# pedroegsilva/gofindthem

Hardware: AMD Instinct MI355X
Metric: ProcessText throughput: documents/s (and input GB/s), 10000-term dictionary + 1000 expressions, 1000000 docs of ~4 KB sharded over 1 GPU(s) (higher is better)
Workload: dtype u8; 1 GPU; BASELINE.json configs[2]: 10000 terms + 1000 AND/OR/NOT expressions, 1000000 docs x ~4 KB on this GPU (SURVEY.md 8(d) generator), case-insensitive finder, inputs resident in HBM; alphabet=lower, keywords=10000, docs_total=1000000, docs_per_gpu=1000000, text_bytes_per_gpu=4100690990, parallelism=docs sharded x1, cu_margin=0

## Files before the change

### gofindthem_amd/csrc/gft_api.cpp

```cpp
#include "../../include/gft.h"

#include <hip/hip_runtime.h>

#include <algorithm>
#include <chrono>
#include <cstdio>
#include <cstring>
#include <map>
#include <memory>
#include <mutex>
#include <string>
#include <thread>
#include <unordered_set>
#include <vector>

#include <cstdlib>

#include "ac_tables.hpp"
#include "copy_pool.hpp"
#include "gft_guard.hpp"
#include "gft_kernels.hpp"
#include "host_solve.hpp"
#include "scan2_tables.hpp"
#include "scan3_tables.hpp"

using namespace gft;

namespace {

struct DevBuf {
    void* p = nullptr;
    size_t cap = 0;
    hipError_t ensure(size_t bytes) {
        if (bytes <= cap) return hipSuccess;
        if (p) { hipError_t e = hipFree(p); p = nullptr; cap = 0; if (e != hipSuccess) return e; }
        size_t want = bytes + bytes / 8 + 256;
        hipError_t e = hipMalloc(&p, want);
        if (e == hipSuccess) cap = want;
        return e;
    }
    void release() { if (p) (void)hipFree(p); p = nullptr; cap = 0; }
    template <class T> T* as() const { return reinterpret_cast<T*>(p); }
};

struct ProfCat {
    std::vector<std::pair<hipEvent_t, hipEvent_t>> ev;
};

}

#ifndef GFT_EXTRA_KERNELS
namespace gft {
bool scan2_plan(uint32_t, uint32_t, uint32_t, uint32_t, size_t, uint32_t*, uint32_t*) { return false; }
hipError_t launch_scan2(const Scan2Params&, uint32_t, unsigned, hipStream_t) { return hipErrorNotSupported; }
bool scan4_plan(uint32_t, uint32_t, uint32_t, uint32_t, size_t, bool, uint32_t*, uint32_t*) { return false; }
hipError_t launch_scan4(const Scan2Params&, uint32_t, unsigned, hipStream_t) { return hipErrorNotSupported; }
}
static constexpr bool kExtraKernels = false;
#else
static constexpr bool kExtraKernels = true;
#endif

struct gft_engine {
    int device = 0;
    hipStream_t stream = nullptr;
    void* pin[2] = {nullptr, nullptr};
    uint64_t* pin_rb = nullptr;
    hipEvent_t pin_ev[2] = {nullptr, nullptr};
    std::unique_ptr<gft::CopyPool> copy_pool;
    bool own_stream = false;
    unsigned n_cus = 256;
    unsigned n_cus_hw = 256, cu_margin = 0;
    size_t lds_max = 65536;
    mutable std::string err;

    AcTables tab;
    bool built = false;
    uint32_t build_flags = 0;
    uint32_t n_lds_states = 0;
    DevBuf d_byte_class, d_delta, d_out_term, d_out_link, d_term_len;
    Scan2Tables s2;
    bool use_scan2 = false;
    DevBuf d_s2_filter, d_s2_slots, d_s2_more, d_s2_cls, d_s2_cls_fold, d_s2_term_blob, d_s2_term_off, d_dbg;
    Scan3Tables s3;
    bool use_scan3 = false;
    DevBuf d_s3_filter, d_s3_short3, d_s3_srec, d_s3_short3_big, d_s3_srec_big, d_s3_bloom, d_s3_slots, d_s3_more, d_s3_cls,
        d_s3_cls_fold, d_s3_term_blob, d_s3_term_off;
    uint32_t scan3_waves = 0, scan3_cand_cap = 0;
    DevBuf d_ctl;
    DevBuf d_s2_short3, d_s2_shorts_packed, d_s2_short3_big, d_s2_fpt;
    uint32_t scan2_short3_bytes = 0;
    uint32_t scan2_k2_waves = 0, scan2_cand_cap = 0;
    bool use_scan4 = false;
    uint32_t scan4_waves = 0, scan4_fifo[2] = {0, 0};
    double scan4_density = 0.06;
    bool use_scan5 = false;
    Scan5Plan s5plan{0, 0, 0, 0};
    Scan5Tables s5;
    DevBuf d_s5_grp, d_s5_grp_fold, d_s5_filter, d_s5_bloom;
    std::vector<uint32_t> s5_bloom;
    uint32_t s5_bloom_lg = 0;
    uint32_t opt_scan5_bloom_kb = 32;
    uint32_t s5_term_bits = 0, s5_pos_bias = 0;
    bool s5_short_groups = false;
    uint32_t opt_scan5_large = 1;
    uint32_t opt_scan5_fifo = 0;
    uint32_t opt_scan5_groups = 0;
    uint64_t scan_valid_docs = ~0ull;
    uint32_t scan2_unit_max = kScan2UnitMax;
    bool deferred = false;
    uint64_t deferred_unit_cap = 0, deferred_pool_cap = 0;
    uint32_t last_nonascii_bits = 0;
    bool last_nonascii = false;
    uint64_t last_text_lo = 0, last_text_hi = 0;
    uint32_t opt_scan_dbg = 0;
    uint32_t opt_scan_prio = 1;
    uint32_t opt_scan_ordered = 0;
    uint32_t opt_scan4_round = 0;
    uint32_t opt_scan4_chunk = 0;
    uint32_t opt_solve_dbg = 0;
    int opt_solve_group = -1;
    mutable std::recursive_mutex mu;
    std::vector<gft_engine*> peers;
    std::vector<uint64_t> shard_cut;
    bool in_multi = false;
    std::vector<void*> comms;
    bool rccl_self = false;
    void* rccl_lib = nullptr;

    bool have_programs = false;
    uint32_t n_exprs = 0, n_extra = 0;
    std::vector<uint32_t> h_prog;
    std::vector<uint64_t> h_prog_off;
    std::vector<ProgramTraits> traits;
    std::vector<uint32_t> host_only;
    std::vector<uint32_t> inord_exprs;
    std::vector<uint8_t> inord_slot;
    uint64_t last_n_units = 0, last_total = 0;
    bool csr_valid = false;
    DevBuf d_patch;
    DevBuf d_prog, d_prog_off;
    DevBuf d_fprog, d_fprog_off, d_groups;
    DevBuf d_wide_slot, d_wide_theta;
    DevBuf d_solve_dbg;
    int single_streak = 0;
    uint64_t last_static_slabs = 0;
    bool deferred_single = false;
    uint32_t ctl_epoch = 1, deferred_epoch = 0;
    uint64_t deferred_n_docs = 0;
    struct Pending {
        bool done = false;
        int rc = 0;
        const uint8_t* d_text = nullptr; const uint64_t* d_doc_off = nullptr; uint64_t n_docs = 0; uint32_t flags = 0;
        uint32_t* d_bitmap = nullptr;
        bool single = false; uint32_t epoch = 0; uint64_t n_docs_cap = 0, unit_cap = 0, pool_cap = 0, static_slabs = 0;
        uint64_t* rb = nullptr; hipEvent_t ev = nullptr;
        bool nonascii = false; uint32_t nonascii_bits = 0; uint64_t text_lo = 0, text_hi = 0;
    };
    Pending pend[2];
    unsigned pend_head = 0, pend_count = 0;
    DevBuf d_order, d_blk_class, d_wave_blk;
    uint32_t last_solve_group_docs = 64;
    DevBuf d_fprog_t, d_fblk_off;
    uint32_t fprog_words = 0;
    uint32_t n_inord_groups = 0;
    uint32_t wide_pairs = 0;
    uint32_t n_wide = 0;
    DevBuf d_wide_list;
    uint32_t n_rare_words = 0;
    DevBuf d_pscratch;

    DevBuf d_unit_cnt, d_unit_base, d_units, d_partial, d_pool_term, d_pool_pos, d_unit_start,
        d_unit_count, d_unit_out, d_term, d_pos, d_match_off;
    uint64_t pool_cap = 0;
    DevBuf d_text, d_doc_off, d_bitmap, d_xoff, d_xslot, d_xpos;
    DevBuf d_uq_first, d_uq_cnt, d_uq_off, d_uq_term;
    DevBuf d_rn_cnt, d_rn_base, d_rn_starts, d_rn_prefix;
    std::vector<uint64_t> h_match_off;
    std::vector<uint32_t> h_term, h_pos;

    int profiling = 0;
    std::vector<hipEvent_t> prof_pool;
    std::map<std::string, ProfCat> prof;
};

namespace {

void refresh_options(gft_engine* e) {
    auto num = [](const char* name, long dflt) { const char* v = getenv(name); return v ? atol(v) : dflt; };
    e->opt_scan_dbg = (uint32_t)num("GFT_SCAN_DEBUG", 0);
    e->opt_scan_prio = num("GFT_SCAN_PRIO", 1) ? 1u : 0u;
    e->opt_scan_ordered = getenv("GFT_SCAN_ORDERED") ? 1u : 0u;
    e->opt_scan4_chunk = (uint32_t)num("GFT_SCAN4_CHUNK", 0);
    e->opt_scan4_round = (uint32_t)num("GFT_SCAN4_ROUND", 0);
    e->opt_scan5_groups = (uint32_t)num("GFT_SCAN5_GROUPS", 0);
    e->opt_scan5_large = num("GFT_SCAN5_LARGE", 1) ? 1u : 0u;
    e->opt_scan5_bloom_kb = (uint32_t)std::min<long>(std::max<long>(num("GFT_SCAN5_BLOOM_KB", 32), 0), 64);
    e->opt_scan5_fifo = (uint32_t)std::min<long>(std::max<long>(num("GFT_SCAN5_FIFO", 0), 0), 4096) & ~63u;
    e->opt_solve_dbg = (uint32_t)num("GFT_SOLVE_DEBUG", 0);
    e->opt_solve_group = (int)num("GFT_SOLVE_GROUP_DOCS", -1);
}
#define GFT_LOCK(e) std::lock_guard<std::recursive_mutex> _gft_lock((e)->mu)

int fail(const gft_engine* e, int code, const std::string& msg) {
    e->err = msg;
    return code;
}
int fail_hip(const gft_engine* e, hipError_t h, const char* what) {
    e->err = std::string(what) + ": " + hipGetErrorString(h);
    return GFT_E_HIP;
}

#define HIP_TRY(expr, what)                                   \
    do {                                                      \
        hipError_t _h = (expr);                               \
        if (_h != hipSuccess) return fail_hip(e, _h, what);   \
    } while (0)

struct DeviceGuard {
    int prev = -1;
    bool ok = true;
    explicit DeviceGuard(int dev) {
        if (hipGetDevice(&prev) != hipSuccess) prev = -1;
        if (prev != dev) ok = hipSetDevice(dev) == hipSuccess;
    }
    ~DeviceGuard() { if (prev >= 0) (void)hipSetDevice(prev); }
};

struct SyncOnExit {
    gft_engine* e;
    explicit SyncOnExit(gft_engine* e_) : e(e_) {}
    ~SyncOnExit() { if (e->device >= 0 && e->stream) (void)hipStreamSynchronize(e->stream); }
};

struct ProfScope {
    gft_engine* e;
    hipEvent_t a = nullptr, b = nullptr;
    ProfScope(gft_engine* e_, const char* cat) : e(e_) {
        if (!e->profiling || (e->profiling == 2 && std::strcmp(cat, "scan") != 0)) return;
        auto get = [&](hipEvent_t* ev) {
            if (!e->prof_pool.empty()) { *ev = e->prof_pool.back(); e->prof_pool.pop_back(); return true; }
            return hipEventCreate(ev) == hipSuccess;
        };
        if (!get(&a) || !get(&b)) { a = b = nullptr; return; }
        (void)hipEventRecord(a, e->stream);
        e->prof[cat].ev.emplace_back(a, b);
    }
    ~ProfScope() { if (b) (void)hipEventRecord(b, e->stream); }
};

template <class T>
int upload(gft_engine* e, DevBuf& buf, const std::vector<T>& v, const char* what) {
    HIP_TRY(buf.ensure(std::max<size_t>(v.size() * sizeof(T), 16)), what);
    if (!v.empty()) HIP_TRY(hipMemcpyAsync(buf.p, v.data(), v.size() * sizeof(T), hipMemcpyHostToDevice, e->stream), what);
    return GFT_OK;
}

int check_program(const gft_engine* e, const uint32_t* w, uint64_t len, uint32_t n_slots, uint32_t idx, ProgramTraits* traits = nullptr) {
    uint32_t sp = 0, psp = 0, g_tot = 0, g_psp = 0, max_sp = 0;
    std::vector<uint32_t> group_slots;
    std::vector<uint32_t> pcnt;
    bool in_group = false;
    auto bad = [&](const char* m) {
        return fail(e, GFT_E_INVALID, "program " + std::to_string(idx) + ": " + m);
    };
    for (uint64_t pc = 0; pc < len; pc++) {
        const uint32_t op = w[pc] >> 28;
        const bool fl = (w[pc] & GFT_INORD_FLAG) != 0;
        switch (op) {
        case GFT_OP_UNIT:
            if ((w[pc] & GFT_SLOT_MASK) >= n_slots) return bad("slot out of range");
            sp++;
            if (fl) { pcnt.push_back(1); in_group = true; group_slots.push_back(w[pc] & GFT_SLOT_MASK); }
            break;
        case GFT_OP_AND:
        case GFT_OP_OR:
            if (sp < 2) return bad("operand stack underflow");
            sp--;
            if (fl) {
                if (pcnt.size() < 2) return bad("INORD operand stack underflow");
                uint32_t r = pcnt.back(); pcnt.pop_back();
                if (op == GFT_OP_AND) pcnt.back() = r; else pcnt.back() += r;
            }
            break;
        case GFT_OP_NOT:
            if (sp < 1) return bad("operand stack underflow");
            if (in_group) return bad("NOT inside INORD");
            break;
        case GFT_OP_INORD:
            if (sp < 1 || pcnt.size() != 1) return bad("malformed INORD group");
            pcnt.clear(); in_group = false;
            if (traits && (g_tot > kMaxPairs || g_psp > kMaxPairDepth) && g_tot <= kMaxPairsWide && g_psp <= kMaxPairDepthWide) {
                traits->wide_pairs = std::max(traits->wide_pairs, g_tot);
                traits->wide_groups.push_back(pc);
            }
            g_tot = g_psp = 0;
            if (traits && group_slots.size() > 1) traits->inord_slots.insert(traits->inord_slots.end(), group_slots.begin(), group_slots.end());
            group_slots.clear();
            break;
        default:
            return bad("unknown opcode");
        }
        max_sp = std::max(max_sp, sp);
        if (sp > kMaxBoolDepth && !traits)
            return fail(e, GFT_E_UNSUPPORTED, "program " + std::to_string(idx) + ": operand stack deeper than " +
                                                   std::to_string(kMaxBoolDepth));
        uint32_t tot = 0;
        for (uint32_t c : pcnt) tot += c;
        psp = (uint32_t)pcnt.size();
        g_tot = std::max(g_tot, tot); g_psp = std::max(g_psp, psp);
        if (tot > kMaxPairs || psp > kMaxPairDepth) {
            if (!traits) return fail(e, GFT_E_UNSUPPORTED, "program " + std::to_string(idx) + ": INORD group too wide for the device solver");
            if (tot > kMaxPairsWide || psp > kMaxPairDepthWide) traits->over_limit = true;
        }
    }
    if (sp != 1 || !pcnt.empty()) return bad("program does not reduce to one value");
    if (traits && traits->wide_pairs && max_sp > kMaxPairDepthWide) traits->over_limit = true;
    if (traits) {
        std::sort(traits->inord_slots.begin(), traits->inord_slots.end());
        traits->inord_slots.erase(std::unique(traits->inord_slots.begin(), traits->inord_slots.end()), traits->inord_slots.end());
    }
    return GFT_OK;
}

uint32_t fuse_program(const uint32_t* w, uint64_t len, uint64_t gbase, std::vector<uint32_t>& out,
                      std::vector<uint32_t>& groups) {
    struct Node { uint32_t op, slot; int64_t l, r; uint64_t s, e; };
    std::vector<Node> nodes;
    std::vector<int64_t> st;
    for (uint64_t i = 0; i < len; i++) {
        const uint32_t op = w[i] >> 28;
        switch (op) {
        case GFT_OP_UNIT:
            nodes.push_back(Node{op, w[i] & GFT_SLOT_MASK, -1, -1, i, i});
            st.push_back((int64_t)nodes.size() - 1);
            break;
        case GFT_OP_AND:
        case GFT_OP_OR: {
            const int64_t r = st.back(); st.pop_back();
            const int64_t l = st.back(); st.pop_back();
            nodes.push_back(Node{op, 0, l, r, nodes[l].s, i});
            st.push_back((int64_t)nodes.size() - 1);
            break;
        }
        case GFT_OP_NOT:
        case GFT_OP_INORD: {
            const int64_t c = st.back(); st.pop_back();
            nodes.push_back(Node{op, 0, c, -1, nodes[c].s, i});
            st.push_back((int64_t)nodes.size() - 1);
            break;
        }
        default:
            break;
        }
    }
    if (st.empty()) return 0;
    const size_t out0 = out.size();
    auto strip = [&](int64_t n, bool& neg) {
        while (nodes[n].op == GFT_OP_NOT) { neg = !neg; n = nodes[n].l; }
        return n;
    };
    std::vector<uint32_t> need(nodes.size(), 0);
    for (size_t n = 0; n < nodes.size(); n++) {
        const Node& nd = nodes[n];
        bool dummy = false;
        if (nd.op == GFT_OP_NOT || nd.op == GFT_OP_INORD) need[n] = need[nd.l];
        else if (nd.op == GFT_OP_AND || nd.op == GFT_OP_OR) {
            const int64_t l = strip(nd.l, dummy), r = strip(nd.r, dummy);
            if (nodes[r].op == GFT_OP_UNIT) need[n] = need[nd.l];
            else if (nodes[l].op == GFT_OP_UNIT) need[n] = need[nd.r];
            else need[n] = need[nd.l] == need[nd.r] ? need[nd.l] + 1 : std::max(need[nd.l], need[nd.r]);
        }
    }
    struct Job { int64_t n; int phase; bool neg; };
    std::vector<Job> jobs{{st.back(), 0, false}};
    uint32_t depth = 0, max_depth = 0;
    while (!jobs.empty()) {
        Job j = jobs.back(); jobs.pop_back();
        bool neg = j.neg;
        const int64_t n = j.phase == 0 ? strip(j.n, neg) : j.n;
        const Node& nd = nodes[n];
        switch (nd.op) {
        case GFT_OP_UNIT:
            out.push_back((neg ? kFopSetN : kFopSet) << 28 | nd.slot);
            break;
        case GFT_OP_INORD:
            if (j.phase == 0) { jobs.push_back({n, 1, neg}); jobs.push_back({nd.l, 0, false}); }
            else {
                if (nodes[nd.l].op != GFT_OP_UNIT) {
                    out.push_back(kFopInord << 28 | (uint32_t)(groups.size() / 2));
                    groups.push_back((uint32_t)(gbase + nodes[nd.l].s));
                    groups.push_back((uint32_t)(nodes[nd.l].e - nodes[nd.l].s + 1));
                }
                if (neg) out.push_back(kFopNot << 28);
            }
            break;
        case GFT_OP_AND:
        case GFT_OP_OR: {
            const bool is_and = (nd.op == GFT_OP_AND) != neg;
            if (j.phase == 0) {
                bool ln = neg, rn = neg;
                const int64_t l = strip(nd.l, ln), r = strip(nd.r, rn);
                if (nodes[r].op == GFT_OP_UNIT) { jobs.push_back({n, 1, neg}); jobs.push_back({nd.l, 0, neg}); }
                else if (nodes[l].op == GFT_OP_UNIT) { jobs.push_back({n, 2, neg}); jobs.push_back({nd.r, 0, neg}); }
                else {
                    const bool left_first = need[nd.l] >= need[nd.r];
                    jobs.push_back({n, 4, neg}); jobs.push_back({left_first ? nd.r : nd.l, 0, neg});
                    jobs.push_back({n, 3, neg}); jobs.push_back({left_first ? nd.l : nd.r, 0, neg});
                }
            } else if (j.phase == 1 || j.phase == 2) {
                bool ln = neg;
                const int64_t leaf = strip(j.phase == 1 ? nd.r : nd.l, ln);
                out.push_back((is_and ? (ln ? kFopAndNS : kFopAndS) : (ln ? kFopOrNS : kFopOrS)) << 28 | nodes[leaf].slot);
            } else if (j.phase == 3) {
                out.push_back(kFopPush << 28);
                max_depth = std::max(max_depth, ++depth);
            } else {
                out.push_back((is_and ? kFopAndPop : kFopOrPop) << 28);
                depth--;
            }
            break;
        }
        default:
            break;
        }
    }
    size_t k = out0;
    for (size_t i = out0; i < out.size(); i++) {
        const uint32_t op = out[i] >> 28, nx = i + 1 < out.size() ? out[i + 1] >> 28 : 0u;
        if (op == kFopPush && (nx == kFopSet || nx == kFopSetN)) {
            out[k++] = (nx == kFopSet ? kFopPushSet : kFopPushSetN) << 28 | (out[i + 1] & 0x0FFFFFFFu);
            i++;
        } else out[k++] = out[i];
    }
    out.resize(k);
    return max_depth;
}

int ensure_pool(gft_engine* e, uint64_t entries) {
    if (entries <= e->pool_cap) return GFT_OK;
    HIP_TRY(e->d_pool_term.ensure(entries * 4), "pool alloc");
    HIP_TRY(e->d_pool_pos.ensure(entries * 4), "pool alloc");
    e->pool_cap = std::min(e->d_pool_term.cap, e->d_pool_pos.cap) / 4;
    return GFT_OK;
}

int csr_from_pool(gft_engine* e, uint64_t n_docs) {
    hipStream_t st = e->stream;
    const uint64_t n_units = e->last_n_units, total = e->last_total;
    HIP_TRY(e->d_term.ensure(std::max<uint64_t>(total, 1) * 4), "result alloc");
    HIP_TRY(e->d_pos.ensure(std::max<uint64_t>(total, 1) * 4), "result alloc");
    HIP_TRY(e->d_unit_out.ensure((n_units + 1) * 8), "unit alloc");
    HIP_TRY(e->d_partial.ensure(scan_partials_needed(std::max(n_units, n_docs)) * 8), "unit alloc");
    ProfScope ps(e, "aux");
    HIP_TRY(launch_exclusive_scan(e->d_unit_count.as<uint32_t>(), n_units, e->d_unit_out.as<uint64_t>(),
                                  e->d_partial.as<uint64_t>(), st), "unit_out scan");
    const bool sort_units = e->use_scan2 || e->use_scan3;
    HIP_TRY(launch_gather(e->d_unit_start.as<uint64_t>(), e->d_unit_count.as<uint32_t>(),
                          e->d_unit_out.as<uint64_t>(), n_units, e->d_pool_term.as<uint32_t>(),
                          e->d_pool_pos.as<uint32_t>(), e->d_term.as<uint32_t>(), e->d_pos.as<uint32_t>(),
                          e->d_unit_base.as<uint64_t>(), n_docs, e->d_match_off.as<uint64_t>(), e->n_cus, st,
                          sort_units ? e->d_units.as<Unit>() : nullptr,
                          e->d_term_len.as<uint32_t>(), (e->build_flags & GFT_POS_END) ? 1u : 0u),
            "gather");
    e->csr_valid = true;
    return GFT_OK;
}

constexpr uint64_t kHostUnitDocs = 1024;

int scan_pipeline(gft_engine* e, const uint8_t* d_text, const uint64_t* d_doc_off, uint64_t n_docs, uint32_t flags,
                  bool need_csr, uint64_t* n_matches, const uint64_t* h_doc_off = nullptr, bool defer_ok = false) {
    hipStream_t st = e->stream;
    *n_matches = 0;
    e->deferred = false;
    e->deferred_single = false;
    e->scan_valid_docs = ~0ull;
    e->csr_valid = false;
    HIP_TRY(e->d_match_off.ensure((n_docs + 1) * 8), "match_off alloc");
    if (n_docs == 0) {
        HIP_TRY(hipMemsetAsync(e->d_match_off.p, 0, 8, st), "memset");
        HIP_TRY(hipStreamSynchronize(st), "sync");
        e->last_n_units = e->last_total = 0;
        e->last_nonascii = false;
        e->last_nonascii_bits = 0;
        e->last_text_lo = e->last_text_hi = 0;
        return GFT_OK;
    }
    const uint32_t warm = e->tab.max_term_len ? e->tab.max_term_len - 1 : 0;
    const uint32_t unit_max = e->use_scan3 ? kScan3UnitMax : e->use_scan4 ? kScan4UnitMax : e->use_scan2 ? e->scan2_unit_max : kTextBuf - warm;

    HIP_TRY(e->d_ctl.ensure(64), "control alloc");
    HIP_TRY(e->d_unit_cnt.ensure(n_docs * 4), "unit alloc");
    HIP_TRY(e->d_unit_base.ensure((n_docs + 1) * 8), "unit alloc");
    HIP_TRY(e->d_partial.ensure(scan_partials_needed(n_docs) * 8), "unit alloc");
    uint64_t n_units = 0, text_lo = 0, text_hi = 0;
    const bool host_units = h_doc_off != nullptr && n_docs <= kHostUnitDocs;
    bool units_single = !host_units && defer_ok && !need_csr && e->single_streak >= 2 && e->pool_cap > 0 &&
                        std::min(std::min(e->d_units.cap / sizeof(Unit), e->d_unit_start.cap / 8), e->d_unit_count.cap / 4) >= n_docs;
    if (units_single && ++e->ctl_epoch < 2) { e->ctl_epoch = 1; units_single = false; }
    if (!units_single) HIP_TRY(hipMemsetAsync(e->d_ctl.p, 0, 32, st), "memset");
    std::vector<uint64_t> hub;
    std::vector<Unit> hun;
    struct DrainIf { gft_engine* e; bool on; ~DrainIf() { if (on && e->stream) (void)hipStreamSynchronize(e->stream); } } drain_units{e, host_units};
    if (host_units) {
        hub.assign(n_docs + 1, 0);
        for (uint64_t d = 0; d < n_docs; d++) {
            if (h_doc_off[d + 1] < h_doc_off[d]) return fail(e, GFT_E_INVALID, "doc_off is not ascending");
            const uint64_t n = h_doc_off[d + 1] - h_doc_off[d];
            if (n > 0xFFFFFFFFull) return fail(e, GFT_E_UNSUPPORTED, "a document is longer than 4 GiB - 1 bytes (positions are 32-bit)");
            const uint64_t k = n <= unit_max ? 1 : (n + unit_max - 1) / unit_max;
            hub[d + 1] = hub[d] + k;
            const uint64_t per = (n + k - 1) / k;
            for (uint64_t i = 0; i < k; i++) {
                uint64_t lo = i * per, hi = lo + per < n ? lo + per : n;
                if (lo > n) lo = n;
                hun.push_back(Unit{(uint32_t)d, (uint32_t)lo, (uint32_t)hi});
            }
        }
        n_units = hub[n_docs]; text_lo = h_doc_off[0]; text_hi = h_doc_off[n_docs];
        HIP_TRY(hipMemcpyAsync(e->d_unit_base.p, hub.data(), (n_docs + 1) * 8, hipMemcpyHostToDevice, st), "unit upload");
    } else if (units_single) {
        ProfScope ps(e, "aux");
        HIP_TRY(launch_units_single(d_doc_off, n_docs, unit_max, e->d_units.as<Unit>(), e->d_unit_base.as<uint64_t>(),
                                    e->d_ctl.as<uint32_t>(), e->ctl_epoch, st), "unit table");
        n_units = n_docs; text_lo = 0; text_hi = ~0ull;
        e->deferred = true; e->deferred_single = true; e->deferred_epoch = e->ctl_epoch;
        e->deferred_unit_cap = n_docs; e->deferred_n_docs = n_docs;
    } else {
        {
            ProfScope ps(e, "aux");
            HIP_TRY(launch_unit_count(d_doc_off, n_docs, unit_max, e->d_unit_cnt.as<uint32_t>(), e->d_ctl.as<uint32_t>(), st), "unit_count");
            HIP_TRY(launch_exclusive_scan(e->d_unit_cnt.as<uint32_t>(), n_docs, e->d_unit_base.as<uint64_t>(),
                                          e->d_partial.as<uint64_t>(), st), "unit scan");
            HIP_TRY(launch_pack_ctl(e->d_unit_base.as<uint64_t>(), d_doc_off, n_docs, e->d_ctl.as<uint64_t>() + 4, st), "unit scan");
        }
        const uint64_t cap_units = std::min(std::min(e->d_units.cap / sizeof(Unit), e->d_unit_start.cap / 8), e->d_unit_count.cap / 4);
        e->deferred = defer_ok && !need_csr && cap_units >= n_docs && e->pool_cap > 0;
        if (e->deferred) {
            n_units = cap_units; text_lo = 0; text_hi = ~0ull;
            e->deferred_unit_cap = cap_units; e->deferred_n_docs = n_docs;
        } else {
            uint64_t rb[7] = {0, 0, 0, 0, 0, 0, 0};
            HIP_TRY(hipMemcpyAsync(rb, e->d_ctl.p, sizeof rb, hipMemcpyDeviceToHost, st), "readback");
            HIP_TRY(hipStreamSynchronize(st), "sync");
            n_units = rb[4]; text_lo = rb[5]; text_hi = rb[6];
            e->single_streak = n_units == n_docs ? e->single_streak + 1 : std::min(e->single_streak, 0);
            const uint32_t bad_doc = (uint32_t)rb[0];
            if (text_hi < text_lo) return fail(e, GFT_E_INVALID, "doc_off is not ascending");
            if (bad_doc) return fail(e, GFT_E_INVALID, "doc_off is not ascending, or a document is longer than 4 GiB - 1 bytes (positions are 32-bit)");
        }
    }

    if (!e->deferred) { e->last_text_lo = text_lo; e->last_text_hi = text_hi; }
    HIP_TRY(e->d_units.ensure(n_units * sizeof(Unit)), "unit alloc");
    HIP_TRY(e->d_unit_start.ensure(n_units * 8), "unit alloc");
    HIP_TRY(e->d_unit_count.ensure(n_units * 4), "unit alloc");
    HIP_TRY(e->d_unit_out.ensure((n_units + 1) * 8), "unit alloc");
    HIP_TRY(e->d_partial.ensure(scan_partials_needed(std::max(n_units, n_docs)) * 8), "unit alloc");
    {
        ProfScope ps(e, "aux");
        if (host_units) {
            if (n_units) HIP_TRY(hipMemcpyAsync(e->d_units.p, hun.data(), n_units * sizeof(Unit), hipMemcpyHostToDevice, st), "unit upload");
        } else if (e->deferred_single) {
        } else if (e->deferred) {
            HIP_TRY(hipMemsetAsync(e->d_units.p, 0, n_units * sizeof(Unit), st), "memset");
            HIP_TRY(launch_unit_fill(d_doc_off, n_docs, e->d_unit_base.as<uint64_t>(), e->d_units.as<Unit>(), unit_max, st, n_units), "unit_fill");
            HIP_TRY(launch_clamp_u64(e->d_unit_base.as<uint64_t>(), n_docs + 1, n_units, st), "unit clamp");
        } else {
            HIP_TRY(launch_unit_fill(d_doc_off, n_docs, e->d_unit_base.as<uint64_t>(), e->d_units.as<Unit>(), unit_max, st), "unit_fill");
        }
    }

    if (e->deferred) e->deferred_pool_cap = e->pool_cap;
    int rc = e->deferred ? GFT_OK : ensure_pool(e, std::max<uint64_t>(1u << 20, (text_hi - text_lo) / 16));
    if (!rc && !e->deferred && (e->use_scan2 || e->use_scan3)) {
        const uint64_t wpw = e->use_scan3 ? e->scan3_waves : e->use_scan4 ? e->scan4_waves : e->use_scan5 ? kScan5Waves : e->scan2_k2_waves;
        const uint64_t min_slab = e->use_scan3 ? 2 * kScan3MinRoom
                                  : e->use_scan4 ? kScan4ChunkUnits * ((uint64_t)(unit_max * e->scan4_density * 1.6) + 49) : 64;
        const uint64_t waves = std::min<uint64_t>(std::max<uint64_t>((n_units + wpw - 1) / wpw, 1), e->n_cus) * wpw;
        rc = ensure_pool(e, 2 * waves * min_slab);
    }
    if (rc) return rc;
    uint64_t total = 0;
    for (int attempt = 0; attempt < 3 && e->use_scan3; attempt++) {
        if (attempt) HIP_TRY(hipMemsetAsync(e->d_ctl.as<uint8_t>() + 8, 0, 16, st), "memset");
        Scan3Params P;
        P.text = d_text; P.doc_off = d_doc_off; P.units = e->d_units.as<Unit>(); P.n_units = n_units; P.text_bytes = text_hi;
        P.fold = (flags & GFT_FOLD_ASCII) ? 1 : 0;
        P.cls = P.fold ? e->d_s3_cls_fold.as<uint8_t>() : e->d_s3_cls.as<uint8_t>();
        P.filter = e->d_s3_filter.as<uint32_t>(); P.filter_words = (uint32_t)e->s3.filter.size();
        P.short3 = e->d_s3_short3.as<uint8_t>(); P.short3_bytes = (uint32_t)e->s3.short3.size();
        P.srec = e->d_s3_srec.as<uint32_t>(); P.srec_words = (uint32_t)e->s3.srec.size();
        P.short3_big = e->s3.short3_big.empty() ? nullptr : e->d_s3_short3_big.as<uint32_t>();
        P.srec_big = e->d_s3_srec_big.as<uint32_t>();
        P.bloom = e->d_s3_bloom.as<uint32_t>(); P.bloom_lg = e->s3.bloom_lg; P.bloom_lds = e->s3.bloom_lg <= kScan3BloomLdsLg ? 1 : 0;
        P.slots = e->d_s3_slots.as<Scan2Slot>(); P.slot_shift = e->s3.slot_shift; P.slot_seed = e->s3.slot_seed;
        P.more = e->d_s3_more.as<Scan2Slot>();
        P.term_blob = e->d_s3_term_blob.as<uint8_t>(); P.term_off = e->d_s3_term_off.as<uint32_t>();
        P.G = e->s3.G; P.grouped = e->s3.grouped ? 1 : 0;
        P.pos_end = (e->build_flags & GFT_POS_END) ? 1 : 0;
        P.want_pos = (need_csr || e->n_inord_groups > 0) ? 1 : 0;
        P.prio = e->opt_scan_prio;
        P.dbg = e->opt_scan_dbg;
        P.nonascii = e->d_ctl.as<uint32_t>() + 6;
        P.cand_cap = e->scan3_cand_cap;
        P.cursor = e->d_ctl.as<uint64_t>() + 1; P.pool_cap = e->pool_cap;
        P.pool_term = e->d_pool_term.as<uint32_t>(); P.pool_pos = e->d_pool_pos.as<uint32_t>();
        P.unit_start = e->d_unit_start.as<uint64_t>(); P.unit_count = e->d_unit_count.as<uint32_t>();
        P.n_matches = e->d_ctl.as<uint64_t>() + 2;
        const uint64_t n_waves = (uint64_t)e->n_cus * e->scan3_waves;
        P.slab = (uint32_t)std::min<uint64_t>(kScan2Slab, std::max<uint64_t>(2 * kScan3MinRoom, e->pool_cap / (2 * n_waves)));
        e->last_static_slabs = std::min<uint64_t>(std::max<uint64_t>((n_units + e->scan3_waves - 1) / e->scan3_waves, 1), e->n_cus) * e->scan3_waves * P.slab;
        {
            ProfScope ps(e, "scan");
            HIP_TRY(launch_scan3(P, e->scan3_waves, e->n_cus, st), "scan kernel launch");
        }
        if (e->deferred) return GFT_OK;
        uint64_t ct[3] = {0, 0, 0};
        HIP_TRY(hipMemcpyAsync(ct, e->d_ctl.as<uint8_t>() + 8, 24, hipMemcpyDeviceToHost, st), "readback");
        HIP_TRY(hipStreamSynchronize(st), "scan kernel");
        const uint64_t cursor = ct[0] + e->last_static_slabs;
        total = ct[1];
        e->last_nonascii_bits = (uint32_t)ct[2]; e->last_nonascii = e->last_nonascii_bits != 0;
        if (cursor <= e->pool_cap) break;
        if (attempt == 2) return fail(e, GFT_E_HIP, "match pool overflow persisted");
        rc = ensure_pool(e, cursor + cursor / 16);
        if (rc) return rc;
    }
    for (int attempt = 0; attempt < 3 && e->use_scan2 && !e->use_scan3; attempt++) {
        if (attempt) HIP_TRY(hipMemsetAsync(e->d_ctl.as<uint8_t>() + 8, 0, 16, st), "memset");
        Scan2Params P;
        P.text = d_text; P.doc_off = d_doc_off; P.units = e->d_units.as<Unit>(); P.n_units = n_units;
        P.filter = e->d_s2_filter.as<uint32_t>(); P.filter_words = (uint32_t)e->s2.filter.size();
        P.hashed = e->s2.hashed ? 1 : 0; P.hash_shift = e->s2.hash_shift;
        P.short3 = e->d_s2_short3.as<uint8_t>(); P.short3_bytes = e->scan2_short3_bytes;
        P.fpt = e->d_s2_fpt.as<uint8_t>(); P.fpt_lg = e->s2.fpt_lg;
        P.shorts_packed = e->d_s2_shorts_packed.as<uint32_t>(); P.shorts_words = (uint32_t)std::min<size_t>(e->s2.shorts_packed.size(), 255 * 3);
        P.short3_big = e->s2.short3_big.empty() ? nullptr : e->d_s2_short3_big.as<uint32_t>();
        P.cand_cap = e->scan2_cand_cap;
        P.slots = e->d_s2_slots.as<Scan2Slot>(); P.slot_shift = e->s2.slot_shift; P.slot_seed = e->s2.slot_seed;
        P.more = e->d_s2_more.as<Scan2Slot>();
        P.text_bytes = text_hi;
        P.fold = (flags & GFT_FOLD_ASCII) ? 1 : 0;
        P.cls = P.fold ? e->d_s2_cls_fold.as<uint8_t>() : e->d_s2_cls.as<uint8_t>();
        P.term_blob = e->d_s2_term_blob.as<uint8_t>(); P.term_off = e->d_s2_term_off.as<uint32_t>();
        P.kp = e->s2.kp; P.pad_class = e->s2.pad_class;
        P.pos_end = (e->build_flags & GFT_POS_END) ? 1 : 0;
        P.cursor = e->d_ctl.as<uint64_t>() + 1; P.pool_cap = e->pool_cap;
        P.pool_term = e->d_pool_term.as<uint32_t>(); P.pool_pos = e->d_pool_pos.as<uint32_t>();
        P.unit_start = e->d_unit_start.as<uint64_t>(); P.unit_count = e->d_unit_count.as<uint32_t>();
        P.n_matches = e->d_ctl.as<uint64_t>() + 2;
        const uint64_t n_waves = (uint64_t)e->n_cus * e->scan2_k2_waves;
        P.slab = (uint32_t)std::min<uint64_t>(kScan2Slab, std::max<uint64_t>(64, e->pool_cap / (2 * n_waves)));
        e->last_static_slabs = std::min<uint64_t>(std::max<uint64_t>((n_units + e->scan2_k2_waves - 1) / e->scan2_k2_waves, 1), e->n_cus) * e->scan2_k2_waves * P.slab;
        P.ordered = (need_csr && e->opt_scan_ordered) ? 1 : 0;
        P.want_pos = (need_csr || e->n_inord_groups > 0) ? 1 : 0;
        P.dbg = e->opt_scan_dbg;
        P.nonascii = e->d_ctl.as<uint32_t>() + 6;
        P.prio = e->opt_scan_prio;
        P.dbg_counters = nullptr;
        if (P.dbg & (2 | 64)) {
            HIP_TRY(e->d_dbg.ensure(128), "debug alloc");
            HIP_TRY(hipMemsetAsync(e->d_dbg.p, 0, 128, st), "memset");
            P.dbg_counters = e->d_dbg.as<uint64_t>();
        }
        if (e->use_scan4) {
            const uint64_t n_waves4 = (uint64_t)e->n_cus * e->scan4_waves;
            P.chunk_units = (uint32_t)std::min<uint64_t>(kScan4ChunkUnits, std::max<uint64_t>(1, n_docs / (n_waves4 * 4)));
            if (e->opt_scan4_chunk) P.chunk_units = std::min<uint32_t>(e->opt_scan4_chunk, kScan4ChunkUnits);
            P.cand_cap = e->scan4_fifo[P.want_pos ? 1 : 0];
            P.bound_q16 = (uint32_t)std::min<double>(e->scan4_density * 1.6 * 65536.0 + 1.0, 4.0e9);
            P.bound_add = 48;
            P.round_c = e->opt_scan4_round ? std::min<uint32_t>(64, std::max<uint32_t>(16, e->opt_scan4_round & ~15u)) : 64;
            const uint64_t chunk_need = (uint64_t)P.chunk_units * (((uint64_t)unit_max * P.bound_q16 >> 16) + P.bound_add);
            P.slab = (uint32_t)std::min<uint64_t>(std::max<uint64_t>(kScan2Slab, 4 * chunk_need), std::max<uint64_t>(chunk_need, e->pool_cap / (2 * n_waves4)));
            const uint64_t n_chunks = (n_units + P.chunk_units - 1) / P.chunk_units;
            e->last_static_slabs = std::min<uint64_t>(std::max<uint64_t>((n_chunks + e->scan4_waves - 1) / e->scan4_waves, 1), e->n_cus) * e->scan4_waves * P.slab;
            ProfScope ps(e, "scan");
            HIP_TRY(launch_scan4(P, e->scan4_waves, e->n_cus, st), "scan kernel launch");
        } else if (e->use_scan5) {
            P.s5_filter = e->d_s5_filter.as<uint64_t>(); P.s5_dual = (uint32_t)e->s5.filter.size();
            P.s5_grp = P.fold ? e->d_s5_grp_fold.as<uint8_t>() : e->d_s5_grp.as<uint8_t>();
            P.s5_G = e->s5.G; P.s5_pad_g = e->s5.pad_group;
            P.s5_fifo_cap = e->s5plan.fifo_cap; P.cand_cap = e->s5plan.cand_cap;
            P.s5_sG = 0; P.s5_sgrp = nullptr; P.s5_srec_big = nullptr;
            if (e->s5_short_groups) {
                P.short3 = e->d_s3_short3.as<uint8_t>(); P.short3_bytes = (uint32_t)e->s3.short3.size();
                P.shorts_packed = e->d_s3_srec.as<uint32_t>(); P.shorts_words = (uint32_t)e->s3.srec.size();
                P.short3_big = e->s3.short3_big.empty() ? nullptr : e->d_s3_short3_big.as<uint32_t>();
                P.s5_srec_big = e->d_s3_srec_big.as<uint32_t>();
                P.s5_sgrp = P.fold ? e->d_s3_cls_fold.as<uint8_t>() : e->d_s3_cls.as<uint8_t>();
                P.s5_sG = e->s3.G;
            }
            P.s5_term_bits = e->s5_term_bits; P.s5_pos_bias = e->s5_pos_bias;
            P.s5_bloom = e->s5_bloom_lg ? e->d_s5_bloom.as<uint32_t>() : nullptr; P.s5_bloom_lg = e->s5_bloom_lg;
            const uint64_t n_waves5 = (uint64_t)e->n_cus * kScan5Waves;
            P.slab = (uint32_t)std::min<uint64_t>(kScan2Slab, std::max<uint64_t>(64, e->pool_cap / (2 * n_waves5)));
            e->last_static_slabs = std::min<uint64_t>(std::max<uint64_t>((n_units + kScan5Waves - 1) / kScan5Waves, 1), e->n_cus) * kScan5Waves * P.slab;
            ProfScope ps(e, "scan");
            HIP_TRY(launch_scan5(P, e->n_cus, st), "scan kernel launch");
        } else {
            ProfScope ps(e, "scan");
            HIP_TRY(launch_scan2(P, e->scan2_k2_waves, e->n_cus, st), "scan kernel launch");
        }
        if (P.dbg & 64) {
            uint64_t t[16];
            HIP_TRY(hipMemcpyAsync(t, e->d_dbg.p, sizeof t, hipMemcpyDeviceToHost, st), "debug read-back");
            HIP_TRY(hipStreamSynchronize(st), "debug read-back");
            if (e->use_scan5) fprintf(stderr, "[gft scan debug] scan5 (G=%u, list %u):\n", e->s5.G, e->s5plan.cand_cap);
            if (e->use_scan4)
                fprintf(stderr, "[gft scan debug] scan4 wave cycles per unit: chunk set-up %.0f, filter %.0f, queue push %.0f, stage A issue %.0f, stage A %.0f, stage B %.0f, flush %.0f, unit records %.0f\n",
                        (double)t[4] / n_units, (double)t[5] / n_units, (double)t[6] / n_units, (double)t[7] / n_units, (double)t[8] / n_units,
                        (double)t[9] / n_units, (double)t[10] / n_units, (double)t[11] / n_units);
            else
            fprintf(stderr, "[gft scan debug] wave cycles per unit: first bytes %.0f, filter %.0f, list %.0f, stage A %.0f (scan5: trips %.0f + stage-B issue and short-term trips %.0f), stage B %.0f, flush %.0f, unit record %.0f\n",
                    (double)t[4] / n_units, (double)t[5] / n_units, (double)t[6] / n_units, (double)(t[7] + t[10]) / n_units, (double)t[10] / n_units, (double)t[7] / n_units,
                    (double)t[8] / n_units, (double)t[9] / n_units, (double)t[11] / n_units);
            double sum = 0;
            for (int k = 4; k < 12; k++) sum += (double)t[k];
            if (t[13]) fprintf(stderr, "[gft scan debug] %llu waves: mean %.0f cycles in all, the slowest %.0f (+%.1f %%)\n", (unsigned long long)t[13],
                               sum / (double)t[13], (double)t[12], 100.0 * ((double)t[12] * (double)t[13] / sum - 1.0));
        }
        if (e->deferred) return GFT_OK;
        uint64_t ct[3] = {0, 0, 0};
        HIP_TRY(hipMemcpyAsync(ct, e->d_ctl.as<uint8_t>() + 8, 24, hipMemcpyDeviceToHost, st), "readback");
        HIP_TRY(hipStreamSynchronize(st), "scan kernel");
        const uint64_t cursor = ct[0] + e->last_static_slabs;
        total = ct[1];
        e->last_nonascii_bits = (uint32_t)ct[2]; e->last_nonascii = e->last_nonascii_bits != 0;
        if (P.dbg & 2) {
            uint64_t c4[4] = {0, 0, 0, 0};
            HIP_TRY(hipMemcpy(c4, e->d_dbg.p, 32, hipMemcpyDeviceToHost), "debug readback");
            fprintf(stderr, "[gft scan debug] units=%llu flagged=%llu sum_of_per_unit_max_lane=%llu to_bucket_table=%llu matches=%llu\n",
                    (unsigned long long)n_units, (unsigned long long)c4[0], (unsigned long long)c4[1],
                    (unsigned long long)c4[2], (unsigned long long)total);
        }
        if (cursor <= e->pool_cap) {
            if (e->use_scan4 && text_hi > text_lo) e->scan4_density = std::max(0.002, (double)total / (double)(text_hi - text_lo));
            if (P.ordered == 0 && text_hi > text_lo) {
                const double per_byte = (double)total / (double)(text_hi - text_lo);
                const double want = per_byte > 0 ? 0.75 * (e->use_scan5 ? e->s5plan.fifo_cap : kScan2FifoCap) / per_byte : (double)kScan2UnitMax;
                uint32_t um = want >= kScan2UnitMax ? kScan2UnitMax : (uint32_t)want & ~255u;
                e->scan2_unit_max = std::max<uint32_t>(512, um);
            }
            break;
        }
        if (attempt == 2) return fail(e, GFT_E_HIP, "match pool overflow persisted");
        rc = ensure_pool(e, cursor + cursor / 16);
        if (rc) return rc;
    }
    for (int attempt = 0; attempt < 3 && !e->use_scan2 && !e->use_scan3; attempt++) {
        if (attempt) HIP_TRY(hipMemsetAsync(e->d_ctl.as<uint8_t>() + 8, 0, 16, st), "memset");
        ScanParams P;
        P.text = d_text; P.doc_off = d_doc_off; P.units = e->d_units.as<Unit>(); P.n_units = n_units;
        P.byte_class = e->d_byte_class.as<uint8_t>(); P.delta = e->d_delta.as<uint32_t>();
        P.out_term = e->d_out_term.as<uint32_t>(); P.out_link = e->d_out_link.as<uint32_t>();
        P.term_len = e->d_term_len.as<uint32_t>();
        P.n_classes = e->tab.n_classes; P.n_states = e->tab.n_states; P.n_lds_states = e->n_lds_states;
        P.max_term_len = e->tab.max_term_len;
        P.pos_end = (e->build_flags & GFT_POS_END) ? 1 : 0;
        P.fold = (flags & GFT_FOLD_ASCII) ? 1 : 0;
        P.nonascii = e->d_ctl.as<uint32_t>() + 6;
        P.cursor = e->d_ctl.as<uint64_t>() + 1; P.pool_cap = e->pool_cap;
        P.pool_term = e->d_pool_term.as<uint32_t>(); P.pool_pos = e->d_pool_pos.as<uint32_t>();
        P.unit_start = e->d_unit_start.as<uint64_t>(); P.unit_count = e->d_unit_count.as<uint32_t>();
        e->last_static_slabs = 0;
        {
            ProfScope ps(e, "scan");
            HIP_TRY(launch_scan_units(P, e->n_cus, st), "scan kernel launch");
        }
        if (e->deferred) return GFT_OK;
        uint64_t ct[3] = {0, 0, 0};
        HIP_TRY(hipMemcpyAsync(ct, e->d_ctl.as<uint8_t>() + 8, 24, hipMemcpyDeviceToHost, st), "readback");
        HIP_TRY(hipStreamSynchronize(st), "scan kernel");
        total = ct[0];
        e->last_nonascii_bits = (uint32_t)ct[2]; e->last_nonascii = e->last_nonascii_bits != 0;
        if (total <= e->pool_cap) break;
        if (attempt == 2) return fail(e, GFT_E_HIP, "match pool overflow persisted");
        rc = ensure_pool(e, total + total / 16);
        if (rc) return rc;
    }

    *n_matches = total;
    e->last_n_units = n_units; e->last_total = total;
    if (!need_csr) return GFT_OK;
    return csr_from_pool(e, n_docs);
}

struct DeferredLaunch { bool single; uint64_t n_docs, unit_cap, pool_cap, static_slabs; uint32_t epoch; };
int deferred_interpret(gft_engine* e, const uint64_t* rb, const DeferredLaunch& dl, bool* again);

int deferred_check(gft_engine* e, bool* again) {
    *again = false;
    if (!e->deferred) return GFT_OK;
    e->deferred = false;
    if (!e->pin_rb) HIP_TRY(hipHostMalloc((void**)&e->pin_rb, 64, hipHostMallocDefault), "pinned alloc");
    uint64_t* rb = e->pin_rb;
    HIP_TRY(hipMemcpyAsync(rb, e->d_ctl.p, 7 * sizeof(uint64_t), hipMemcpyDeviceToHost, e->stream), "readback");
    HIP_TRY(hipStreamSynchronize(e->stream), "process pipeline");
    return deferred_interpret(e, rb, DeferredLaunch{e->deferred_single, e->deferred_n_docs, e->deferred_unit_cap, e->deferred_pool_cap, e->last_static_slabs, e->deferred_single ? e->deferred_epoch : 0u}, again);
}

int deferred_interpret(gft_engine* e, const uint64_t* rb, const DeferredLaunch& dl, bool* again) {
    *again = false;
    const uint64_t cursor = rb[1] + dl.static_slabs, total = rb[2], n_units = rb[4], text_lo = rb[5], text_hi = rb[6];
    e->last_nonascii_bits = (uint32_t)rb[3]; e->last_nonascii = e->last_nonascii_bits != 0;
    const bool flag_bad = dl.single ? (uint32_t)rb[0] == dl.epoch : (uint32_t)rb[0] != 0;
    if (dl.single && (uint32_t)(rb[3] >> 32) == dl.epoch) {
        e->single_streak = -8;
        *again = true;
        return GFT_OK;
    }
    e->single_streak = n_units == dl.n_docs ? e->single_streak + 1 : std::min(e->single_streak, 0);
    e->last_text_lo = text_lo; e->last_text_hi = text_hi;
    e->last_n_units = n_units; e->last_total = total;
    if (text_hi < text_lo) return fail(e, GFT_E_INVALID, "doc_off is not ascending");
    if (flag_bad) return fail(e, GFT_E_INVALID, "doc_off is not ascending, or a document is longer than 4 GiB - 1 bytes (positions are 32-bit)");
    if (n_units > dl.unit_cap || cursor > dl.pool_cap) {
        if (cursor > dl.pool_cap) { int rc = ensure_pool(e, cursor + cursor / 16); if (rc) return rc; }
        *again = true;
        return GFT_OK;
    }
    if (e->use_scan4 && text_hi > text_lo) e->scan4_density = std::max(0.002, (double)total / (double)(text_hi - text_lo));
    if (e->use_scan2 && !e->use_scan3 && !e->opt_scan_ordered && text_hi > text_lo) {
        const double per_byte = (double)total / (double)(text_hi - text_lo);
        const double want = per_byte > 0 ? 0.75 * (e->use_scan5 ? e->s5plan.fifo_cap : kScan2FifoCap) / per_byte : (double)kScan2UnitMax;
        const uint32_t um = want >= kScan2UnitMax ? kScan2UnitMax : (uint32_t)want & ~255u;
        e->scan2_unit_max = std::max<uint32_t>(512, um);
    }
    return GFT_OK;
}

int refine_nonascii(gft_engine* e, const uint8_t* d_text, const uint64_t* d_doc_off, uint64_t n_docs, uint32_t flags) {
    if (!(flags & GFT_FOLD_ASCII)) { e->last_nonascii = false; return GFT_OK; }
    if (!e->last_nonascii) return GFT_OK;
    if (!(e->last_nonascii_bits & 1u)) { e->last_nonascii = (e->last_nonascii_bits & 2u) != 0; return GFT_OK; }
    uint32_t flag = 0;
    {
        ProfScope ps(e, "aux");
        HIP_TRY(hipMemsetAsync(e->d_ctl.as<uint32_t>() + 6, 0, 4, e->stream), "memset");
        HIP_TRY(launch_fold_safe(d_text, e->last_text_lo, e->last_text_hi, d_doc_off, n_docs, e->d_ctl.as<uint32_t>() + 6, e->stream), "fold check");
    }
    HIP_TRY(hipMemcpyAsync(&flag, e->d_ctl.as<uint32_t>() + 6, 4, hipMemcpyDeviceToHost, e->stream), "readback");
    HIP_TRY(hipStreamSynchronize(e->stream), "fold check");
    e->last_nonascii = (flag & 2u) != 0;
    return GFT_OK;
}

bool pend_settled(const gft_engine* e) {
    for (unsigned i = 0; i < e->pend_count; i++)
        if (!e->pend[(e->pend_head + i) % 2].done) return false;
    return true;
}

int unique_pipeline(gft_engine* e, uint64_t n_docs, uint64_t* n_matches) {
    if (!n_docs) return GFT_OK;
    hipStream_t st = e->stream;
    const uint32_t n_terms = std::max<uint32_t>((uint32_t)e->tab.terms.size(), 1);
    const unsigned grid = (unsigned)std::max<uint64_t>(1, std::min<uint64_t>(std::min<uint64_t>(n_docs, (uint64_t)e->n_cus * 4), (256ull << 20) / ((uint64_t)n_terms * 4)));
    HIP_TRY(e->d_uq_first.ensure((size_t)grid * n_terms * 4), "unique alloc");
    HIP_TRY(e->d_uq_cnt.ensure(n_docs * 4), "unique alloc");
    HIP_TRY(e->d_uq_off.ensure((n_docs + 1) * 8), "unique alloc");
    HIP_TRY(e->d_partial.ensure(scan_partials_needed(n_docs) * 8), "unique alloc");
    HIP_TRY(hipMemsetAsync(e->d_uq_first.p, 0xFF, (size_t)grid * n_terms * 4, st), "memset");
    ProfScope ps(e, "aux");
    HIP_TRY(launch_unique_terms(false, e->d_match_off.as<uint64_t>(), e->d_term.as<uint32_t>(), n_docs, n_terms, e->d_uq_first.as<uint32_t>(), grid,
                                e->d_uq_cnt.as<uint32_t>(), nullptr, nullptr, st), "unique count");
    HIP_TRY(launch_exclusive_scan(e->d_uq_cnt.as<uint32_t>(), n_docs, e->d_uq_off.as<uint64_t>(), e->d_partial.as<uint64_t>(), st), "unique scan");
    uint64_t total = 0;
    HIP_TRY(hipMemcpyAsync(&total, e->d_uq_off.as<uint64_t>() + n_docs, 8, hipMemcpyDeviceToHost, st), "readback");
    HIP_TRY(hipStreamSynchronize(st), "unique scan");
    HIP_TRY(e->d_uq_term.ensure(std::max<uint64_t>(total, 1) * 4), "unique alloc");
    HIP_TRY(launch_unique_terms(true, e->d_match_off.as<uint64_t>(), e->d_term.as<uint32_t>(), n_docs, n_terms, e->d_uq_first.as<uint32_t>(), grid,
                                nullptr, e->d_uq_off.as<uint64_t>(), e->d_uq_term.as<uint32_t>(), st), "unique write");
    std::swap(e->d_match_off, e->d_uq_off);
    std::swap(e->d_term, e->d_uq_term);
    HIP_TRY(e->d_pos.ensure(std::max<uint64_t>(total, 1) * 4), "unique alloc");
    HIP_TRY(hipMemsetAsync(e->d_pos.p, 0, std::max<uint64_t>(total, 1) * 4, st), "memset");
    *n_matches = total;
    return GFT_OK;
}

int rune_pipeline(gft_engine* e, const uint8_t* d_text, const uint64_t* d_doc_off, uint64_t n_docs, uint64_t n_matches) {
    if (!n_docs || !n_matches) return GFT_OK;
    hipStream_t st = e->stream;
    HIP_TRY(e->d_rn_cnt.ensure(n_docs * 4), "rune alloc");
    HIP_TRY(e->d_rn_base.ensure((n_docs + 1) * 8), "rune alloc");
    HIP_TRY(e->d_partial.ensure(scan_partials_needed(n_docs) * 8), "rune alloc");
    ProfScope ps(e, "aux");
    HIP_TRY(launch_rune_doc_blocks(d_doc_off, n_docs, e->d_rn_cnt.as<uint32_t>(), st), "rune blocks");
    HIP_TRY(launch_exclusive_scan(e->d_rn_cnt.as<uint32_t>(), n_docs, e->d_rn_base.as<uint64_t>(), e->d_partial.as<uint64_t>(), st), "rune scan");
    uint64_t n_blocks = 0;
    HIP_TRY(hipMemcpyAsync(&n_blocks, e->d_rn_base.as<uint64_t>() + n_docs, 8, hipMemcpyDeviceToHost, st), "readback");
    HIP_TRY(hipStreamSynchronize(st), "rune scan");
    HIP_TRY(e->d_rn_starts.ensure(std::max<uint64_t>(n_blocks, 1) * 4), "rune alloc");
    HIP_TRY(e->d_rn_prefix.ensure((n_blocks + 1) * 8), "rune alloc");
    HIP_TRY(e->d_partial.ensure(scan_partials_needed(std::max(n_blocks, n_docs)) * 8), "rune alloc");
    HIP_TRY(launch_rune_block_starts(d_text, d_doc_off, e->d_rn_base.as<uint64_t>(), n_docs, n_blocks, e->d_rn_starts.as<uint32_t>(), st), "rune starts");
    HIP_TRY(launch_exclusive_scan(e->d_rn_starts.as<uint32_t>(), n_blocks, e->d_rn_prefix.as<uint64_t>(), e->d_partial.as<uint64_t>(), st), "rune scan");
    HIP_TRY(launch_pos_to_rune(d_text, d_doc_off, e->d_rn_base.as<uint64_t>(), e->d_rn_prefix.as<uint64_t>(), e->d_match_off.as<uint64_t>(), n_docs,
                               n_matches, e->d_pos.as<uint32_t>(), st), "rune offsets");
    return GFT_OK;
}

int solve_pipeline(gft_engine* e, uint64_t n_docs, const gft_extra_matches* d_extra, uint32_t* d_bitmap) {
    if (!n_docs || !e->n_exprs) return GFT_OK;
    SolveParams S;
    S.doc_unit_base = e->d_unit_base.as<uint64_t>();
    S.unit_start = e->d_unit_start.as<uint64_t>(); S.unit_count = e->d_unit_count.as<uint32_t>();
    S.units = e->d_units.as<Unit>();
    S.has_rare = e->n_rare_words > 0 ? 1u : 0u;
    S.pos_back = (e->build_flags & GFT_POS_END) ? 0u : (e->tab.max_term_len ? e->tab.max_term_len - 1 : 0u);
    S.term = e->d_pool_term.as<uint32_t>(); S.pos = e->d_pool_pos.as<uint32_t>();
    S.x_off = d_extra ? d_extra->off : nullptr;
    S.x_slot = d_extra ? d_extra->slot : nullptr;
    S.x_pos = d_extra ? d_extra->pos : nullptr;
    S.n_docs = n_docs;
    S.fprog = e->d_fprog.as<uint32_t>(); S.fprog_off = e->d_fprog_off.as<uint64_t>();
    S.gprog = e->d_prog.as<uint32_t>(); S.groups = e->d_groups.as<uint32_t>();
    S.order = e->d_order.as<uint32_t>(); S.blk_class = e->d_blk_class.as<uint32_t>(); S.wave_blk = e->d_wave_blk.as<uint32_t>();
    S.fprog_t = e->d_fprog_t.as<uint32_t>(); S.fblk_off = e->d_fblk_off.as<uint32_t>();
    S.n_exprs = e->n_exprs;
    S.n_slots = (uint32_t)e->tab.terms.size() + e->n_extra + 1;
    S.tile_words = std::min<uint32_t>(kSolveTileWords, (e->n_exprs + 31) / 32);
    S.bitmap = d_bitmap;
    S.p_scratch = nullptr;
    S.dbg = e->opt_solve_dbg;
    S.dbg_out = nullptr;
    if (S.dbg & 8) {
        HIP_TRY(e->d_solve_dbg.ensure(128 * 8), "debug alloc");
        HIP_TRY(hipMemsetAsync(e->d_solve_dbg.p, 0, 128 * 8, e->stream), "memset");
        S.dbg_out = e->d_solve_dbg.as<unsigned long long>();
    }
    S.fprog_words = e->fprog_words;
    uint32_t group_docs = 64;
    bool p_in_lds = false;
    for (uint32_t G : {64u, 32u, 16u, 8u}) {
        if (e->opt_solve_group >= 0 && (uint32_t)e->opt_solve_group != G) continue;
        if (solve_lds_bytes(S.n_slots, S.tile_words, G, true, 0, 0, false) + 1024 <= e->lds_max) { group_docs = G; p_in_lds = true; break; }
    }
    const bool prog_in_lds = !e->wide_pairs && solve_lds_bytes(S.n_slots, S.tile_words, group_docs, p_in_lds, S.fprog_words, S.n_exprs, true) + 1024 <= e->lds_max;
    const uint64_t n_groups = (n_docs + group_docs - 1) / group_docs;
    const size_t lds_need = solve_lds_bytes(S.n_slots, S.tile_words, group_docs, p_in_lds, S.fprog_words, S.n_exprs, prog_in_lds) + 512;
    const unsigned per_cu = (unsigned)std::max<size_t>(1, std::min<size_t>(8, e->lds_max / lds_need));
    unsigned grid = (unsigned)std::min<uint64_t>(n_groups, (uint64_t)e->n_cus * per_cu);
    if (!p_in_lds) {
        HIP_TRY(e->d_pscratch.ensure((size_t)grid * S.n_slots * 8), "presence scratch alloc");
        S.p_scratch = e->d_pscratch.as<uint64_t>();
    }
    S.wide_slot = nullptr; S.wide_theta = nullptr; S.wide_cap = 0; S.wide_list = nullptr; S.n_wide = 0;
    if (e->wide_pairs) {
        const uint64_t n_waves = (uint64_t)grid * (kSolveBlockThreads / 64);
        S.wide_cap = (e->wide_pairs + 63u) & ~63u;
        HIP_TRY(e->d_wide_slot.ensure(n_waves * S.wide_cap * 4), "INORD scratch alloc");
        HIP_TRY(e->d_wide_theta.ensure(n_waves * S.wide_cap * 8), "INORD scratch alloc");
        S.wide_slot = e->d_wide_slot.as<uint32_t>();
        S.wide_theta = e->d_wide_theta.as<long long>();
        S.wide_list = e->d_wide_list.as<uint32_t>(); S.n_wide = e->n_wide;
    }
    e->last_solve_group_docs = p_in_lds ? group_docs : 0;
    ProfScope ps(e, "solve");
    HIP_TRY(launch_solve(S, group_docs, p_in_lds, prog_in_lds, grid, e->stream), "solve kernel launch");
    if (S.dbg & 8) {
        unsigned long long t[128];
        HIP_TRY(hipMemcpyAsync(t, e->d_solve_dbg.p, sizeof t, hipMemcpyDeviceToHost, e->stream), "debug read-back");
        HIP_TRY(hipStreamSynchronize(e->stream), "debug read-back");
        fprintf(stderr, "[gft solve debug] cycles per group: wave | build bar eval bar transpose bar rows head\n");
        for (int w = 0; w < 16; w++) {
            fprintf(stderr, "[gft solve debug] %2d |", w);
            for (int ph = 0; ph < 8; ph++) fprintf(stderr, " %7.0f", (double)t[w * 8 + ph] / (double)n_groups);
            fprintf(stderr, "\n");
        }
    }
    return GFT_OK;
}

struct HostPlan {
    bool all_docs = false;
    std::vector<uint64_t> irregular;
    bool empty() const { return !all_docs && irregular.empty(); }
};

void plan_host(const gft_engine* e, const gft_extra_matches* extra, uint64_t n_docs, HostPlan& plan) {
    plan.all_docs = !e->host_only.empty();
    plan.irregular.clear();
    if (!extra || !extra->off || e->inord_exprs.empty() || !n_docs) return;
    const uint32_t n_terms = (uint32_t)e->tab.terms.size();
    std::vector<std::pair<uint32_t, uint32_t>> seen;
    for (uint64_t d = 0; d < n_docs; d++) {
        seen.clear();
        bool irr = false;
        for (uint64_t i = extra->off[d]; i < extra->off[d + 1] && !irr; i++) {
            const uint32_t sl = extra->slot[i];
            if (sl >= e->inord_slot.size() || !e->inord_slot[sl]) continue;
            if (sl < n_terms) { irr = true; break; }
            size_t k = 0;
            while (k < seen.size() && seen[k].first != sl) k++;
            if (k == seen.size()) seen.emplace_back(sl, extra->pos[i]);
            else { irr = extra->pos[i] < seen[k].second; seen[k].second = extra->pos[i]; }
        }
        if (irr) plan.irregular.push_back(d);
    }
}

int host_eval(gft_engine* e, const gft_extra_matches* extra, uint64_t n_docs, const HostPlan& plan, uint32_t* h_bitmap,
              uint32_t* d_bitmap) {
    if (plan.empty() || !n_docs || !e->n_exprs) return GFT_OK;
    hipStream_t st = e->stream;
    if (!e->csr_valid) { int rc = csr_from_pool(e, n_docs); if (rc) return rc; }
    std::vector<uint64_t> mo(n_docs + 1);
    HIP_TRY(hipMemcpyAsync(mo.data(), e->d_match_off.p, (n_docs + 1) * 8, hipMemcpyDeviceToHost, st), "download");
    HIP_TRY(hipStreamSynchronize(st), "host solve");
    std::vector<uint64_t> docs;
    if (plan.all_docs) { docs.resize(n_docs); for (uint64_t d = 0; d < n_docs; d++) docs[d] = d; }
    else docs = plan.irregular;
    std::vector<uint32_t> ti, po;
    std::vector<uint64_t> at(docs.size() + 1, 0);
    for (size_t k = 0; k < docs.size(); k++) at[k + 1] = at[k] + (mo[docs[k] + 1] - mo[docs[k]]);
    ti.resize(at.back() + 1); po.resize(at.back() + 1);
    if (plan.all_docs) {
        if (at.back()) {
            HIP_TRY(hipMemcpyAsync(ti.data(), e->d_term.p, at.back() * 4, hipMemcpyDeviceToHost, st), "download");
            HIP_TRY(hipMemcpyAsync(po.data(), e->d_pos.p, at.back() * 4, hipMemcpyDeviceToHost, st), "download");
        }
    } else {
        for (size_t k = 0; k < docs.size(); k++) {
            const uint64_t n = at[k + 1] - at[k];
            if (!n) continue;
            HIP_TRY(hipMemcpyAsync(ti.data() + at[k], e->d_term.as<uint32_t>() + mo[docs[k]], n * 4, hipMemcpyDeviceToHost, st), "download");
            HIP_TRY(hipMemcpyAsync(po.data() + at[k], e->d_pos.as<uint32_t>() + mo[docs[k]], n * 4, hipMemcpyDeviceToHost, st), "download");
        }
    }
    HIP_TRY(hipStreamSynchronize(st), "host solve");
    const uint64_t words = (e->n_exprs + 31) / 32;
    std::vector<uint64_t> pw;
    std::vector<uint32_t> pclr, pset;
    SlotLists lists;
    size_t ir = 0;
    for (size_t k = 0; k < docs.size(); k++) {
        const uint64_t d = docs[k];
        while (ir < plan.irregular.size() && plan.irregular[ir] < d) ir++;
        const bool irregular = ir < plan.irregular.size() && plan.irregular[ir] == d;
        lists.clear();
        for (uint64_t i = at[k]; i < at[k + 1]; i++) lists[ti[i]].push_back((int64_t)po[i]);
        if (extra && extra->off)
            for (uint64_t i = extra->off[d]; i < extra->off[d + 1]; i++) lists[extra->slot[i]].push_back((int64_t)extra->pos[i]);
        auto solve_one = [&](uint32_t x) {
            const bool hit = host_solve(e->h_prog.data() + e->h_prog_off[x], e->h_prog_off[x + 1] - e->h_prog_off[x], lists);
            const uint64_t w = d * words + (x >> 5);
            const uint32_t bit = 1u << (x & 31);
            if (h_bitmap) h_bitmap[w] = hit ? h_bitmap[w] | bit : h_bitmap[w] & ~bit;
            else { pw.push_back(w); pclr.push_back(hit ? 0u : bit); pset.push_back(hit ? bit : 0u); }
        };
        for (uint32_t x : e->host_only) solve_one(x);
        if (irregular) for (uint32_t x : e->inord_exprs) solve_one(x);
    }
    if (!h_bitmap && !pw.empty()) {
        if (!d_bitmap) return fail(e, GFT_E_INVALID, "null bitmap");
        const size_t n = pw.size();
        HIP_TRY(e->d_patch.ensure(n * 16), "patch alloc");
        uint8_t* base = e->d_patch.as<uint8_t>();
        HIP_TRY(hipMemcpyAsync(base, pw.data(), n * 8, hipMemcpyHostToDevice, st), "patch upload");
        HIP_TRY(hipMemcpyAsync(base + n * 8, pclr.data(), n * 4, hipMemcpyHostToDevice, st), "patch upload");
        HIP_TRY(hipMemcpyAsync(base + n * 12, pset.data(), n * 4, hipMemcpyHostToDevice, st), "patch upload");
        HIP_TRY(launch_patch_words(d_bitmap, reinterpret_cast<const uint64_t*>(base), reinterpret_cast<const uint32_t*>(base + n * 8),
                                   reinterpret_cast<const uint32_t*>(base + n * 12), n, st), "patch");
        HIP_TRY(hipStreamSynchronize(st), "patch");
    }
    return GFT_OK;
}

}

namespace {
constexpr uint32_t kTablesMagic = 0x54544647u;
constexpr uint32_t kTablesVersion = 9;

struct Writer {
    std::vector<uint8_t> b;
    void raw(const void* p, size_t n) { const uint8_t* q = (const uint8_t*)p; b.insert(b.end(), q, q + n); }
    void u32(uint32_t v) { raw(&v, 4); }
    void u64(uint64_t v) { raw(&v, 8); }
    template <class T> void vec(const std::vector<T>& v) { u64(v.size()); if (!v.empty()) raw(v.data(), v.size() * sizeof(T)); }
};
struct Reader {
    const uint8_t* p; uint64_t n, i = 0; bool ok = true;
    bool raw(void* d, size_t k) { if (!ok || k > n - i) { ok = false; return false; } memcpy(d, p + i, k); i += k; return true; }
    uint32_t u32() { uint32_t v = 0; raw(&v, 4); return v; }
    uint64_t u64() { uint64_t v = 0; raw(&v, 8); return v; }
    template <class T> void vec(std::vector<T>& v) {
        const uint64_t k = u64();
        if (!ok || k > (n - i) / sizeof(T)) { ok = false; return; }
        v.resize((size_t)k);
        if (k) raw(v.data(), (size_t)k * sizeof(T));
    }
};
const char* validate_tables(const AcTables& a, const Scan2Tables& t, const Scan3Tables& u) {
    const size_t n_terms = a.terms.size();
    if (a.n_classes == 0 || a.n_classes > 256) return "class count";
    for (int b = 0; b < 256; b++) if (a.byte_class[b] >= a.n_classes) return "byte class";
    for (uint32_t d : a.delta) if ((d & ~kOutFlag) >= a.n_states) return "DFA target";
    for (uint32_t x : a.out_term) if (x != kNoTerm && x >= n_terms) return "DFA output term";
    for (uint32_t x : a.out_link) if (x >= a.n_states) return "DFA output link";
    for (size_t i = 0; i < n_terms; i++) if (a.term_len[i] != a.terms[i].size()) return "term length";
    auto slots_ok = [&](const std::vector<Scan2Slot>& slots, const std::vector<Scan2Slot>& more, uint32_t shift, const std::vector<uint8_t>& blob,
                        const std::vector<uint32_t>& off) -> const char* {
        if (shift < 1 || shift > 31 || slots.size() != ((size_t)1 << (32 - shift))) return "bucket table size";
        if (off.size() != n_terms + 1) return "term offsets";
        for (size_t i = 0; i < n_terms; i++)
            if (off[i] < 4 || (uint64_t)off[i] + a.terms[i].size() + 8 > blob.size()) return "term offset";
        auto entry_ok = [&](const Scan2Slot& s) {
            const uint32_t len1 = s.len & kScan2LenMask;
            const int off8 = (int)(int8_t)(s.len >> 24);
            return s.info < n_terms && off8 >= -1 && off8 <= (int)kScan2MaxOff && (int64_t)len1 + off8 == (int64_t)a.terms[s.info].size() && len1 >= 4;
        };
        for (const Scan2Slot& s : slots) {
            if (s.key == kScan2EmptyKey) continue;
            if (s.info & kScan2Multi) {
                const uint64_t at = s.info & ~kScan2Multi;
                if (at + s.len > more.size() || s.len == 0) return "bucket list";
            } else if (!entry_ok(s)) return "bucket entry";
        }
        for (const Scan2Slot& s : more) if (s.key != kScan2EmptyKey && !entry_ok(s)) return "bucket list entry";
        return nullptr;
    };
    if (t.supported) {
        if (t.kp == 0 || t.kp > 256 || t.pad_class >= t.kp) return "scan2 classes";
        for (int b = 0; b < 256; b++) if (t.cls[b] >= t.kp || t.cls_fold[b] >= t.kp) return "scan2 byte class";
        if (t.kp != a.n_classes) return "scan2 class count differs from the automaton's";
        for (int b = 0; b < 256; b++) if (t.cls[b] != a.byte_class[b]) return "scan2 byte class differs from the automaton's";
        if (t.slot_shift < 1 || t.slot_shift > 31) return "bucket table size";
        for (size_t i = 0; i < t.slots.size(); i++)
// ... 1511 lines not shown
```

### gofindthem_amd/csrc/gft_kernels.hpp

```cpp
#pragma once
#include <hip/hip_runtime.h>
#include <stdint.h>

namespace gft {

constexpr uint32_t kScanBlockThreads = 512;
constexpr uint32_t kTextBuf = 8448;
constexpr uint32_t kSolveBlockThreads = 1024;
constexpr uint32_t kMaxPairs = 64;
constexpr uint32_t kMaxPairDepth = 32;
constexpr uint32_t kMaxBoolDepth = 128;
constexpr uint32_t kMaxPairsWide = 8192;
constexpr uint32_t kMaxPairDepthWide = 64;

#define GFT_K_INORD_FLAG (1u << 27)
#define GFT_K_SLOT_MASK ((1u << 27) - 1u)

struct Unit { uint32_t doc, lo, hi; };

struct ScanParams {
    const uint8_t* text;
    const uint64_t* doc_off;
    const Unit* units;
    uint64_t n_units;
    const uint8_t* byte_class;
    const uint32_t* delta;
    const uint32_t* out_term;
    const uint32_t* out_link;
    const uint32_t* term_len;
    uint32_t n_classes, n_states, n_lds_states, max_term_len;
    uint32_t pos_end, fold;
    uint32_t* nonascii;
    uint64_t* cursor;
    uint64_t pool_cap;
    uint32_t* pool_term;
    uint32_t* pool_pos;
    uint64_t* unit_start;
    uint32_t* unit_count;
};

enum FusedOp : uint32_t {
    kFopSet = 1,
    kFopAndS = 2,
    kFopOrS = 3,
    kFopSetN = 5,
    kFopAndNS = 6,
    kFopOrNS = 7,
    kFopAndPop = 8,
    kFopOrPop = 9,
    kFopNot = 10,
    kFopInord = 11,
    kFopPush = 12,
    kFopNop = 13,
    kFopPushSet = 14,
    kFopPushSetN = 15
};
constexpr uint32_t kSolveRegStack = 2;
constexpr uint32_t kSolveRegStackDeep = 4;

constexpr uint32_t kDwNeg = 1u << 0, kDwSel = 1u << 1, kDwOnes = 1u << 2, kDwOr = 1u << 28, kDwPop = 1u << 29,
                   kDwPush = 1u << 30, kDwRare = 1u << 31;
constexpr uint32_t kDwFieldShift = 3, kDwFieldBits = 25;
constexpr uint32_t kDwFieldMask = ((1u << kDwFieldBits) - 1u) << kDwFieldShift;
constexpr uint32_t kDwNop = kDwOnes;
inline uint32_t fused_to_device(uint32_t fw) {
    const uint32_t field = (fw << kDwFieldShift) & kDwFieldMask;
    switch (fw >> 28) {
    case kFopSet: return field | kDwOr;
    case kFopSetN: return field | kDwOr | kDwNeg;
    case kFopAndS: return field | kDwSel;
    case kFopAndNS: return field | kDwSel | kDwNeg;
    case kFopOrS: return field | kDwOnes | kDwOr;
    case kFopOrNS: return field | kDwOnes | kDwOr | kDwNeg;
    case kFopAndPop: return kDwPop | kDwSel;
    case kFopOrPop: return kDwPop | kDwOnes | kDwOr;
    case kFopPush: return kDwPush | kDwOnes;
    case kFopPushSet: return field | kDwPush | kDwOr;
    case kFopPushSetN: return field | kDwPush | kDwOr | kDwNeg;
    case kFopNot: return kDwRare | kDwOnes | kDwNeg;
    case kFopInord: return kDwRare | kDwOnes | field;
    default: return kDwNop;
    }
}
constexpr uint32_t kSolveTileWords = 64;

struct SolveParams {
    const uint64_t* doc_unit_base;
    const uint64_t* unit_start;
    const uint32_t* unit_count;
    const uint32_t* term;
    const uint32_t* pos;
    const uint64_t* x_off;
    const uint32_t* x_slot;
    const uint32_t* x_pos;
    uint64_t n_docs;
    const uint32_t* fprog;
    const uint64_t* fprog_off;
    const uint32_t* gprog;
    const uint32_t* groups;
    const uint32_t* order;
    const Unit* units;
    uint32_t has_rare;
    uint32_t pos_back;
    const uint32_t* blk_class;
    const uint32_t* wave_blk;
    const uint32_t* fprog_t;
    const uint32_t* fblk_off;
    uint32_t n_exprs, n_slots, tile_words;
    uint32_t fprog_words;
    uint32_t dbg;
    unsigned long long* dbg_out;
    uint64_t* p_scratch;
    uint32_t* wide_slot;
    long long* wide_theta;
    uint32_t wide_cap;
    const uint32_t* wide_list;
    uint32_t n_wide;
    uint32_t* bitmap;
};

#if defined(__HIPCC__)
#define GFT_HD __host__ __device__
#else
#define GFT_HD
#endif

constexpr uint32_t kScan2Threads = 1024;
constexpr uint32_t kScan2StageCap = 6;
constexpr uint32_t kScan2FifoCap = 256;
constexpr uint32_t kScan2CandCapMin = 512;
constexpr uint32_t kScan2Slab = 4096;
constexpr uint32_t kScan2UnitMax = 8192;
constexpr uint32_t kGoldDev = 0x9E3779B1u;

constexpr uint32_t kScan2EmptyKey = 0xFFFFFFFFu;
constexpr uint32_t kScan2Multi = 0x80000000u;
constexpr uint32_t kScan2InlineLen = 24;
constexpr uint32_t kScan2MaxOff = 4;
constexpr uint32_t kScan2LenMask = 0x00FFFFFFu;
struct __attribute__((aligned(32))) Scan2Slot {
    uint32_t key;
    uint32_t info;
    uint32_t len;
    uint32_t front[5];
};
struct Scan2Short {
    uint32_t n;
    uint32_t term[3];
    uint32_t len[3];
    uint32_t pad;
};
constexpr uint32_t kScan2Short3Max = 32768;
constexpr uint32_t kScan2FptSize = 20480;
constexpr uint32_t kScan2FptLdsItems = 11000;
constexpr uint32_t kScan2FptAmbiguous = 0xFF;
template <uint32_t C>
GFT_HD inline uint32_t scan2_mul24c(uint32_t a) {
#if defined(__HIP_DEVICE_COMPILE__)
    uint32_t d;
    asm("v_mul_u32_u24 %0, %1, %2" : "=v"(d) : "n"(C), "v"(a));
    return d;
#else
    return (uint32_t)((uint64_t)(a & 0xFFFFFFu) * (uint64_t)(C & 0xFFFFFFu));
#endif
}
GFT_HD inline uint32_t scan2_slot_hash(uint32_t x, int which, uint32_t shift, uint32_t seed) {
    const uint32_t xf = (x ^ (x >> 20)) + seed;
    return (which ? scan2_mul24c<0x85EBCBu>(xf) : scan2_mul24c<0x9E3779u>(xf)) >> shift;
}
GFT_HD inline uint32_t scan2_pair_slot(uint32_t x, int which, uint32_t shift, uint32_t seed) {
    const uint32_t xf = (x ^ (x >> 20)) + seed;
    return ((scan2_mul24c<0x9E3779u>(xf) >> shift) & ~1u) | (uint32_t)which;
}
GFT_HD inline uint32_t scan2_fpt_index(uint32_t h, uint32_t fpt_lg) {
    return fpt_lg ? h >> (32 - fpt_lg) : scan2_mul24c<kScan2FptSize>(h >> 16) >> 16;
}
GFT_HD inline uint32_t scan2_fpt_xcell(uint32_t x, uint32_t fpt_lg) { return scan2_fpt_index(scan2_mul24c<0x3779B1u>(x), fpt_lg); }
GFT_HD inline uint32_t scan2_fpt_gcell(uint32_t x, uint32_t b1n, int which, uint32_t fpt_lg) {
    return scan2_fpt_index(which ? scan2_mul24c<0xB2AE35u>(x) + scan2_mul24c<0x9E4F2Du>(b1n)
                                 : scan2_mul24c<0xC2B2AFu>(x) + scan2_mul24c<0x27D4EBu>(b1n), fpt_lg);
}
GFT_HD inline uint32_t scan2_fpt_xmix(uint32_t x) { return scan2_mul24c<0xD4EB2Fu>(x); }
GFT_HD inline uint32_t scan2_fpt_xbyte(uint32_t xmix) { return 1u + (xmix >> 25); }
GFT_HD inline bool scan2_fpt_pass(uint32_t cx, uint32_t cg0, uint32_t cg1, uint32_t xmix, uint32_t tw) {
    (void)tw;
    const uint32_t tag = scan2_fpt_xbyte(xmix);
    const bool amb = (cx == kScan2FptAmbiguous) | (cg0 == kScan2FptAmbiguous) | (cg1 == kScan2FptAmbiguous);
    return (cx == tag) | (cg0 == tag) | (cg1 == tag) | amb;
}

struct Scan2Params {
    const uint8_t* text;
    const uint64_t* doc_off;
    const Unit* units;
    uint64_t n_units;
    const uint32_t* filter;
    uint32_t filter_words, hashed, hash_shift;
    const uint8_t* short3;
    uint32_t short3_bytes;
    const uint32_t* shorts_packed;
    uint32_t shorts_words;
    const uint32_t* short3_big;
    uint32_t cand_cap;
    const uint8_t* fpt;
    uint32_t fpt_lg;
    const Scan2Slot* slots;
    uint32_t slot_shift, slot_seed;
    const Scan2Slot* more;
    const uint8_t* cls;
    const uint8_t* term_blob;
    const uint32_t* term_off;
    uint32_t kp, pad_class, fold, pos_end;
    uint64_t* cursor;
    uint64_t pool_cap;
    uint32_t* pool_term;
    uint32_t* pool_pos;
    uint64_t* unit_start;
    uint32_t* unit_count;
    uint64_t* n_matches;
    uint32_t slab;
    uint32_t ordered;
    uint64_t text_bytes;
    uint32_t prio;
    uint32_t want_pos;
    uint32_t dbg;
    uint32_t* nonascii;
    uint64_t* dbg_counters;
    uint32_t chunk_units;
    uint32_t bound_q16, bound_add;
    uint32_t round_c;
    const uint8_t* s5_grp;
    uint32_t s5_G, s5_pad_g;
    const uint64_t* s5_filter;
    uint32_t s5_dual;
    uint32_t s5_fifo_cap;
    const uint8_t* s5_sgrp;
    uint32_t s5_sG;
    const uint32_t* s5_srec_big;
    uint32_t s5_term_bits, s5_pos_bias;
    const uint32_t* s5_bloom;
    uint32_t s5_bloom_lg;
};
GFT_HD inline uint32_t scan5_bloom_g(uint32_t x, uint32_t b1n, uint32_t lg) {
    return (scan2_mul24c<0xC2B2AFu>(x ^ (x >> 20)) + scan2_mul24c<0x27D4EBu>(b1n + 1)) >> (32 - lg);
}
GFT_HD inline uint32_t scan5_bloom_x(uint32_t x, uint32_t lg) { return scan2_mul24c<0x3779B1u>(x ^ (x >> 20)) >> (32 - lg); }
bool scan2_plan(uint32_t filter_words, uint32_t short3_bytes, uint32_t shorts_words, uint32_t fpt_lds_bytes, size_t lds_max,
                uint32_t* waves, uint32_t* cand_cap);
hipError_t launch_scan2(const Scan2Params& P, uint32_t waves, unsigned n_cus, hipStream_t st);
constexpr uint32_t kScan4ChunkUnits = 8;
constexpr uint32_t kScan4UnitMax = 8176;
bool scan4_plan(uint32_t filter_words, uint32_t short3_bytes, uint32_t shorts_words, uint32_t fpt_lds_bytes, size_t lds_max, bool want_pos,
                uint32_t* waves, uint32_t* fifo_cap);
hipError_t launch_scan4(const Scan2Params& P, uint32_t waves, unsigned n_cus, hipStream_t st);
constexpr uint32_t kScan5Waves = 16;
constexpr uint32_t kScan5MaxGroups = 27;
constexpr uint32_t kScan5SurvX = 64;
constexpr uint32_t kScan5CandCapMin = 384;
struct Scan5Plan { uint32_t G, dual_entries, cand_cap, fifo_cap; };
bool scan5_plan(uint32_t kp, uint32_t short3_bytes, uint32_t shorts_words, uint32_t fpt_lds_bytes, size_t lds_max, uint32_t fifo_cap, Scan5Plan* out);
hipError_t launch_scan5(const Scan2Params& P, unsigned n_cus, hipStream_t st);


constexpr uint32_t kScan3Groups = 27;
constexpr uint32_t kScan3Threads = 1024;
constexpr uint32_t kScan3UnitMax = 8192;
constexpr uint32_t kScan3RecWords = 6;
constexpr uint32_t kScan3RecLds = 254;
constexpr uint32_t kScan3BloomLdsLg = 13;
constexpr uint32_t kScan3SurvCap = 128;
constexpr uint32_t kScan3MinRoom = 512;
constexpr uint32_t kScan3CandCapMin = 256;
constexpr uint32_t kScan3BloomMul1 = 0x9E3779B1u, kScan3BloomMul2 = 0x85EBCA6Bu;
GFT_HD inline uint32_t scan3_bloom_cell(uint32_t key5, uint32_t lg) { return (key5 * kScan3BloomMul1) >> (32 - lg); }
GFT_HD inline uint32_t scan3_bloom_bits(uint32_t key5) {
    const uint32_t h = key5 * kScan3BloomMul2;
    return 1u << (h >> 27) | 1u << ((h >> 22) & 31);
}

struct Scan3Params {
    const uint8_t* text;
    const uint64_t* doc_off;
    const Unit* units;
    uint64_t n_units;
    uint64_t text_bytes;
    const uint8_t* cls;
    const uint32_t* filter;
    uint32_t filter_words;
    const uint8_t* short3;
    uint32_t short3_bytes;
    const uint32_t* srec;
    uint32_t srec_words;
    const uint32_t* short3_big;
    const uint32_t* srec_big;
    const uint32_t* bloom;
    uint32_t bloom_lg, bloom_lds;
    const Scan2Slot* slots;
    uint32_t slot_shift, slot_seed;
    const Scan2Slot* more;
    const uint8_t* term_blob;
    const uint32_t* term_off;
    uint32_t G, fold, pos_end, want_pos, grouped, prio;
    uint32_t cand_cap;
    uint32_t dbg;
    uint32_t* nonascii;
    uint64_t* cursor;
    uint64_t pool_cap;
    uint32_t* pool_term;
    uint32_t* pool_pos;
    uint64_t* unit_start;
    uint32_t* unit_count;
    uint64_t* n_matches;
    uint32_t slab;
};
bool scan3_plan(uint32_t filter_words, uint32_t short3_bytes, uint32_t srec_words, uint32_t bloom_lds_bytes, size_t lds_max,
                uint32_t* waves, uint32_t* cand_cap);
hipError_t launch_scan3(const Scan3Params& P, uint32_t waves, unsigned n_cus, hipStream_t st);

hipError_t launch_unit_count(const uint64_t* d_doc_off, uint64_t n_docs, uint32_t unit_max, uint32_t* d_cnt,
                             uint32_t* d_bad, hipStream_t st);
hipError_t launch_pack_ctl(const uint64_t* d_unit_base, const uint64_t* d_doc_off, uint64_t n_docs, uint64_t* d_out, hipStream_t st);
hipError_t launch_unit_fill(const uint64_t* d_doc_off, uint64_t n_docs, const uint64_t* d_unit_base, Unit* d_units,
                            uint32_t unit_max, hipStream_t st, uint64_t max_units = ~0ull);
hipError_t launch_units_single(const uint64_t* d_doc_off, uint64_t n_docs, uint32_t unit_max, Unit* d_units, uint64_t* d_unit_base,
                               uint32_t* d_ctl32, uint32_t epoch, hipStream_t st);
hipError_t launch_patch_words(uint32_t* d_words, const uint64_t* d_idx, const uint32_t* d_clr, const uint32_t* d_set, uint64_t n, hipStream_t st);
hipError_t launch_clamp_u64(uint64_t* d_v, uint64_t n, uint64_t cap, hipStream_t st);
uint64_t scan_partials_needed(uint64_t n);
hipError_t launch_exclusive_scan(const uint32_t* d_in, uint64_t n, uint64_t* d_out, uint64_t* d_partial,
                                 hipStream_t st);
size_t scan_units_lds_bytes(uint32_t n_lds_states, uint32_t n_classes);
hipError_t launch_scan_units(const ScanParams& P, unsigned n_cus, hipStream_t st);
hipError_t launch_gather(const uint64_t* d_unit_start, const uint32_t* d_unit_count, const uint64_t* d_unit_out,
                         uint64_t n_units, const uint32_t* d_pool_term, const uint32_t* d_pool_pos, uint32_t* d_term,
                         uint32_t* d_pos, const uint64_t* d_unit_base, uint64_t n_docs, uint64_t* d_match_off,
                         unsigned n_cus, hipStream_t st, const Unit* d_units_to_sort = nullptr,
                         const uint32_t* d_term_len = nullptr, uint32_t pos_end = 0);
hipError_t launch_fold_safe(const uint8_t* d_text, uint64_t lo, uint64_t hi, const uint64_t* d_doc_off, uint64_t n_docs, uint32_t* d_flag, hipStream_t st);
hipError_t launch_unique_terms(bool write, const uint64_t* d_match_off, const uint32_t* d_term, uint64_t n_docs, uint32_t n_terms,
                               uint32_t* d_first, unsigned grid, uint32_t* d_cnt, const uint64_t* d_out_off, uint32_t* d_out_term,
                               hipStream_t st);
hipError_t launch_rune_doc_blocks(const uint64_t* d_doc_off, uint64_t n_docs, uint32_t* d_cnt, hipStream_t st);
hipError_t launch_rune_block_starts(const uint8_t* d_text, const uint64_t* d_doc_off, const uint64_t* d_blk_base, uint64_t n_docs,
                                    uint64_t n_blocks, uint32_t* d_starts, hipStream_t st);
hipError_t launch_pos_to_rune(const uint8_t* d_text, const uint64_t* d_doc_off, const uint64_t* d_blk_base, const uint64_t* d_blk_prefix,
                              const uint64_t* d_match_off, uint64_t n_docs, uint64_t n_matches, uint32_t* d_pos, hipStream_t st);
size_t solve_lds_bytes(uint32_t n_slots, uint32_t tile_words, uint32_t group_docs, bool p_in_lds, uint32_t prog_words,
                       uint32_t n_exprs, bool prog_in_lds);
hipError_t launch_solve(const SolveParams& S, uint32_t group_docs, bool p_in_lds, bool prog_in_lds, unsigned grid, hipStream_t st);

}
```

### gofindthem_amd/csrc/gft_scan5.hip

```cpp
#include <hip/hip_runtime.h>

#include <cstdlib>

#include "gft_kernels.hpp"

namespace gft {


namespace {

#include "gft_scan2_dev.hpp"
#include "gft_foldsafe_dev.hpp"

constexpr int kWays5 = 2;

struct Ctx5 {
    uint32_t* fifo;
    uint32_t fifo_cap;
    uint32_t nf;
    uint32_t npend;
    bool lost;
    bool direct;
    uint64_t dbase;
    uint32_t term_bits, pos_base;
};

__device__ __forceinline__ void out_append(const Scan2Params& P, Ctx5& o, bool em, uint32_t term, uint32_t pos) {
    const uint64_t mask = __ballot(em);
    if (em) {
        const uint32_t idx = o.nf + __builtin_amdgcn_mbcnt_hi((uint32_t)(mask >> 32), __builtin_amdgcn_mbcnt_lo((uint32_t)mask, 0));
        if (!o.direct) {
            if (idx < o.fifo_cap - o.npend) o.fifo[idx] = P.want_pos ? term | (pos - o.pos_base) << o.term_bits : term;
        } else {
            KARG(pool_term)[o.dbase + idx] = term;
            if (P.want_pos) KARG(pool_pos)[o.dbase + idx] = pos;
        }
    }
    o.nf += (uint32_t)__popcll(mask);
    if (!o.direct && o.nf + o.npend > o.fifo_cap) o.lost = true;
}

__device__ __forceinline__ void wave_lds_sync() {
    __builtin_amdgcn_fence(__ATOMIC_RELEASE, "wavefront");
    __builtin_amdgcn_wave_barrier();
    __builtin_amdgcn_fence(__ATOMIC_ACQUIRE, "wavefront");
}

__device__ __forceinline__ void short_trip(const Ctx& c, Ctx5& o, uint32_t ubase, uint32_t n) {
    const uint32_t lane = lane_id();
    const bool on = lane < n;
    const uint32_t job = o.fifo[o.fifo_cap - 1 - (o.npend - n) - (on ? lane : 0)];
    o.npend -= n;
    const uint32_t p = ubase + (job & 0xFFFFu), sid = on ? job >> 16 : 0;
    uint32_t r[3] = {0, 0, 0};
    if (sid) {
        const uint32_t* src = c.lrec + 3 * sid;
        r[0] = src[0]; r[1] = src[1]; r[2] = src[2];
    }
#pragma unroll
    for (uint32_t j = 0; j < 3; j++) {
        if (j && !__any(r[j] != 0)) break;
        const uint32_t L = r[j] >> 28;
        out_append(c.P, o, r[j] != 0 && L <= p + 1, r[j] & 0x0FFFFFFFu, c.P.pos_end ? p : p + 1 - L);
    }
}
__device__ __forceinline__ void park_short(const Ctx& c, Ctx5& o, uint32_t ubase, uint32_t rel, uint32_t sid, uint32_t x3) {
    if (!__any(sid != 0)) return;
    if (__builtin_expect(__any(sid == 255) && KARG(short3_big) != nullptr, 0)) {
        uint32_t r[3] = {0, 0, 0};
        const uint32_t p = ubase + rel;
        if (sid) short_record(c, sid, x3, r);
#pragma unroll
        for (uint32_t j = 0; j < 3; j++) {
            const uint32_t L = r[j] >> 28;
            out_append(c.P, o, r[j] != 0 && L <= p + 1, r[j] & 0x0FFFFFFFu, c.P.pos_end ? p : p + 1 - L);
        }
        return;
    }
    const uint64_t m = __ballot(sid != 0);
    const uint32_t n = (uint32_t)__popcll(m);
    if (o.npend + n > o.fifo_cap / 2) {
        wave_lds_sync();
        while (o.npend) short_trip(c, o, ubase, o.npend < 64 ? o.npend : 64);
        wave_lds_sync();
    }
    if (!o.direct && o.nf + o.npend + n > o.fifo_cap) o.lost = true;
    if (sid) o.fifo[o.fifo_cap - 1 - o.npend - __builtin_amdgcn_mbcnt_hi((uint32_t)(m >> 32), __builtin_amdgcn_mbcnt_lo((uint32_t)m, 0))] = rel | sid << 16;
    o.npend += n;
}

__device__ __forceinline__ void short_trip_g(const Ctx& c, Ctx5& o, lds_u8* lsg, uint32_t ubase, uint32_t n) {
    const Scan2Params& P = c.P;
    const uint32_t lane = lane_id();
    const bool on = lane < n;
    const uint32_t job = o.fifo[o.fifo_cap - 1 - (o.npend - n) - (on ? lane : 0)];
    o.npend -= n;
    const uint32_t p = ubase + (job & 0xFFFFu);
    uint32_t sid = on ? job >> 16 : 0;
    const Text8 t8 = cand_load(c, p);
    const uint32_t W = P.fold ? fold4(t8.w) : t8.w;
    if (__builtin_expect(__any(sid == 255), 0)) {
        const uint32_t G = P.s5_sG;
        const uint32_t x3 = (lsg[(t8.w >> 8) & 0xFF] * G + lsg[(t8.w >> 16) & 0xFF]) * G + lsg[t8.w >> 24];
        const bool b = sid == 255;
        uint32_t cnt = 0;
        const uint32_t* g = nullptr;
        if (b) { g = KARG(s5_srec_big) + KARG(short3_big)[x3]; cnt = g[0]; }
        for (uint32_t j = 0; __any(j < cnt); j++) {
            uint32_t w0 = 0, w1 = 0;
            if (j < cnt) { w0 = g[1 + 2 * j]; w1 = g[2 + 2 * j]; }
            const uint32_t L = w0 >> 28;
            const bool ok = w0 != 0 && L <= p + 1 && ((W ^ w1) >> ((32 - 8 * L) & 31)) == 0;
            out_append(P, o, ok, w0 & 0x0FFFFFFFu, P.pos_end ? p : p + 1 - L);
        }
        if (b) sid = 0;
    }
    if (!__any(sid != 0)) return;
    const uint32_t* r = c.lrec + sid * kScan3RecWords;
#pragma unroll
    for (uint32_t j = 0; j < 3; j++) {
        const uint32_t w0 = sid ? r[2 * j] : 0;
        if (j && !__any(w0 != 0)) break;
        const uint32_t L = w0 >> 28;
        const bool ok = w0 != 0 && L <= p + 1 && ((W ^ r[2 * j + 1]) >> ((32 - 8 * L) & 31)) == 0;
        out_append(P, o, ok, w0 & 0x0FFFFFFFu, P.pos_end ? p : p + 1 - L);
    }
}
__device__ __forceinline__ void park_short_g(const Ctx& c, Ctx5& o, lds_u8* lsg, uint32_t ubase, uint32_t rel, uint32_t sid) {
    if (!__any(sid != 0)) return;
    const uint64_t m = __ballot(sid != 0);
    const uint32_t n = (uint32_t)__popcll(m);
    if (o.npend + n > o.fifo_cap / 2) {
        wave_lds_sync();
        while (o.npend) short_trip_g(c, o, lsg, ubase, o.npend < 64 ? o.npend : 64);
        wave_lds_sync();
    }
    if (!o.direct && o.nf + o.npend + n > o.fifo_cap) o.lost = true;
    if (sid) o.fifo[o.fifo_cap - 1 - o.npend - __builtin_amdgcn_mbcnt_hi((uint32_t)(m >> 32), __builtin_amdgcn_mbcnt_lo((uint32_t)m, 0))] = rel | sid << 16;
    o.npend += n;
}

__device__ __forceinline__ void finish_long5(const Ctx& c, Ctx5& o, bool on, uint32_t rel, const Cand& k, const Slot& s0, const Slot& s1,
                                             Front t, uint32_t tl, Deferred& d) {
    const Scan2Params& P = c.P;
    Slot e;
    const bool have = slot_pick(k.x, s0, s1, e) && on;
    if (!__any(have)) return;
    const bool multi = have && (e.a.y & kScan2Multi);
    uint32_t folded = 0;
    {
        const bool act = have && !multi;
        const uint32_t kmax = wave_kmax(act ? e.a.z & kScan2LenMask : 0);
        if (P.fold) front_fold_upto(t, folded, kmax);
        const bool ok = act && entry_ok(c, k.p, t, tl, e, kmax);
        out_append(P, o, ok, e.a.y, match_pos(P, k.p, e.a.z));
    }
    if (!__any(multi)) return;
    const uint32_t n_ent = multi ? e.a.z : 0, more_at = e.a.y & ~kScan2Multi;
    const uint32_t tot = lane_value(wave_incl_scan(n_ent), 63);
    if (tot <= d.cap - d.n) {
        for (uint32_t j = 0; __any(j < n_ent); j++) {
            const uint64_t m = __ballot(j < n_ent);
            if (j < n_ent)
                d.list[d.n + __builtin_amdgcn_mbcnt_hi((uint32_t)(m >> 32), __builtin_amdgcn_mbcnt_lo((uint32_t)m, 0))] =
                    make_uint2(rel, more_at + j);
            d.n += (uint32_t)__popcll(m);
        }
        return;
    }
    Slot cur = e;
    if (multi) cur = slot_load(&P.more[more_at]);
    for (uint32_t j = 0; __any(j < n_ent); j++) {
        const bool act = j < n_ent;
        Slot nxt = cur;
        if (j + 1 < n_ent) nxt = slot_load(&P.more[more_at + j + 1]);
        const uint32_t kmax = wave_kmax(act ? cur.a.z & kScan2LenMask : 0);
        if (P.fold) front_fold_upto(t, folded, kmax);
        const bool ok = act && entry_ok(c, k.p, t, tl, cur, kmax);
        out_append(P, o, ok, cur.a.y, match_pos(P, k.p, cur.a.z));
        cur = nxt;
    }
}


__device__ __forceinline__ void drain_deferred5(const Ctx& c, Ctx5& o, uint32_t ubase, Deferred& d) {
    const Scan2Params& P = c.P;
    const uint32_t lane = lane_id();
    wave_lds_sync();
    for (uint32_t i0 = 0; i0 < d.n; i0 += 64) {
        const bool on = i0 + lane < d.n;
        const uint2 it = d.list[on ? i0 + lane : 0];
        const uint32_t p = ubase + it.x;
        const Slot e = slot_load(&P.more[it.y]);
        const Text8 t8 = cand_load(c, p);
        Front t = front_load(c, p, t8.tw);
        const uint32_t tl = tail_load(c, p);
        const uint32_t kmax = wave_kmax(on ? e.a.z & kScan2LenMask : 0);
        uint32_t folded = 0;
        if (P.fold) front_fold_upto(t, folded, kmax);
        const bool ok = on && entry_ok(c, p, t, tl, e, kmax);
        out_append(P, o, ok, e.a.y, match_pos(P, p, e.a.z));
    }
    d.n = 0;
    __builtin_amdgcn_wave_barrier();
}

template <bool FPT_LDS, bool DBG, bool SG>
__global__ void __launch_bounds__(kScan2Threads) k_scan5(const Scan2Params P) {
    extern __shared__ __align__(16) uint8_t smem[];
    uint8_t* grp = smem;
    uint8_t* cls = smem + 256;
    uint8_t* sgrp = smem + 512;
    uint64_t* dual = reinterpret_cast<uint64_t*>(smem + 768);
    uint8_t* short3 = reinterpret_cast<uint8_t*>(dual + P.s5_dual);
    uint8_t* fpt = short3 + P.short3_bytes;
    const uint32_t bloom_lg = FPT_LDS ? 0u : __builtin_amdgcn_readfirstlane(P.s5_bloom_lg);
    const uint32_t bloom_bytes = bloom_lg ? (1u << bloom_lg) / 8 : 0u;
    uint32_t* lrec = reinterpret_cast<uint32_t*>(fpt + (FPT_LDS ? kScan2FptSize : bloom_bytes));
    uint32_t* wg_next = reinterpret_cast<uint32_t*>(smem + (((size_t)(reinterpret_cast<uint8_t*>(lrec) - smem) + P.shorts_words * 4 + 15) & ~(size_t)15));
    uint8_t* wave_lds_all = reinterpret_cast<uint8_t*>(wg_next) + 16;

    for (uint32_t i = threadIdx.x; i < 256; i += blockDim.x) { grp[i] = P.s5_grp[i]; cls[i] = P.cls[i]; sgrp[i] = SG ? P.s5_sgrp[i] : 0; }
    for (uint32_t i = threadIdx.x; i < P.s5_dual; i += blockDim.x) dual[i] = P.s5_filter[i];
    for (uint32_t i = threadIdx.x; i < P.short3_bytes / 4; i += blockDim.x)
        reinterpret_cast<uint32_t*>(short3)[i] = reinterpret_cast<const uint32_t*>(P.short3)[i];
    for (uint32_t i = threadIdx.x; FPT_LDS && i < kScan2FptSize / 4; i += blockDim.x)
        reinterpret_cast<uint32_t*>(fpt)[i] = reinterpret_cast<const uint32_t*>(P.fpt)[i];
    for (uint32_t i = threadIdx.x; !FPT_LDS && i < bloom_bytes / 4; i += blockDim.x) reinterpret_cast<uint32_t*>(fpt)[i] = P.s5_bloom[i];
    for (uint32_t i = threadIdx.x; i < P.shorts_words; i += blockDim.x) lrec[i] = P.shorts_packed[i];
    if (threadIdx.x == 0) { wg_next[0] = kScan5Waves; wg_next[1] = wg_next[2] = wg_next[3] = 0; }
    __syncthreads();
    if (DBG && (P.dbg & 128)) return;

    const uint32_t lane = lane_id(), wave = __builtin_amdgcn_readfirstlane(threadIdx.x >> 6);
    uint8_t* wave_lds = wave_lds_all + (size_t)wave * (P.s5_fifo_cap * 4 + kScan5SurvX * 4 + ((P.cand_cap * 2 + 15) & ~15u));
    uint32_t* fifo = reinterpret_cast<uint32_t*>(wave_lds);
    uint32_t* survx = fifo + P.s5_fifo_cap;
    uint16_t* cand = reinterpret_cast<uint16_t*>(survx + kScan5SurvX);
    const uint32_t G = __builtin_amdgcn_readfirstlane(P.s5_G);
    const uint32_t kp = __builtin_amdgcn_readfirstlane(P.kp), kp2 = __builtin_amdgcn_readfirstlane(kp * kp);
    lds_u8* lgrp = (lds_u8*)0;
    typedef uint32_t u32x2 __attribute__((ext_vector_type(2)));
    typedef __attribute__((address_space(3))) const u32x2 lds_u64;
    lds_u64* ldual = (lds_u64*)768;
    lds_u8* lsg = (lds_u8*)512;
    if ((uint32_t)(uintptr_t)(lds_u8*)smem != 0) __builtin_trap();

    unsigned long long tl[8] = {0, 0, 0, 0, 0, 0, 0, 0}, tprev = DBG ? clock64() : 0;
    auto mark = [&](int ph) {
        if (DBG && (P.dbg & 64)) { const unsigned long long now = clock64(); tl[ph] += now - tprev; tprev = now; }
    };
    auto static_slabs = [&]() { return (uint64_t)gridDim.x * kScan5Waves * KARG(slab); };
    uint64_t slab_next = ((uint64_t)blockIdx.x * kScan5Waves + wave) * KARG(slab);
    uint32_t wave_matches = 0;
    bool told_nonascii = false;
    uint32_t slab_left = KARG(slab);

    constexpr uint32_t wg_waves = kScan5Waves;
    const uint64_t round_units = (uint64_t)gridDim.x * wg_waves, wg_first = (uint64_t)blockIdx.x * wg_waves;
    auto unit_of = [&](uint32_t item) -> uint64_t { return (uint64_t)(item / wg_waves) * round_units + wg_first + item % wg_waves; };
    uint64_t u = unit_of(wave), nu = 0;
    Unit un_n{0, 0, 0};
    uint64_t abs_n = 0, end_n = 0;
    if (u < P.n_units) { un_n = P.units[u]; abs_n = P.doc_off[un_n.doc]; end_n = P.doc_off[un_n.doc + 1]; }
    for (; u < P.n_units; u = nu) {
        const Unit un{(uint32_t)__builtin_amdgcn_readfirstlane(un_n.doc), (uint32_t)__builtin_amdgcn_readfirstlane(un_n.lo),
                      (uint32_t)__builtin_amdgcn_readfirstlane(un_n.hi)};
        const uint64_t doc_abs = (uint64_t)(uint32_t)__builtin_amdgcn_readfirstlane((uint32_t)(abs_n >> 32)) << 32 |
                                 (uint32_t)__builtin_amdgcn_readfirstlane((uint32_t)abs_n);
        const uint64_t end_v = end_n;
        {
            uint32_t item = 0;
            if (lane == 0) item = __hip_atomic_fetch_add(wg_next, 1u, __ATOMIC_RELAXED, __HIP_MEMORY_SCOPE_WORKGROUP);
            nu = unit_of((uint32_t)__builtin_amdgcn_readfirstlane(item));
        }
        mark(7);
        const bool more_units = nu < P.n_units;
        if (more_units) un_n = P.units[nu];
        const Ctx c{P, cls, nullptr, P.short3_bytes ? short3 : nullptr, fpt, lrec, P.text + doc_abs, doc_abs, kp2,
                    doc_abs < 7, doc_abs < 23, un.lo, un.hi, doc_abs + un.hi + 4 > P.text_bytes, DBG ? P.dbg : 0u};
        const uint32_t nborder = un.lo < kScan2MaxOff ? un.lo : kScan2MaxOff;
        const uint32_t ubase = un.lo - kScan2MaxOff;
        const uint32_t own = un.hi - un.lo;
        const uint32_t C = ((own + 63) / 64 + 3) & ~3u;
        const uint32_t my_lo = un.lo + lane * C;
        const uint32_t my_hi = my_lo + C < un.hi ? my_lo + C : un.hi;
        const uint32_t nvalid = my_lo < un.hi ? my_hi - my_lo : 0;
        Ctx5 o{fifo, P.s5_fifo_cap, 0, 0, false, false, 0, P.s5_term_bits, un.lo - P.s5_pos_bias};

        uint32_t m0 = 0, m1 = 0, m2 = 0, m3 = 0;
        if (own) {
            uint32_t h1 = P.s5_pad_g, h2 = P.s5_pad_g, h3 = P.s5_pad_g, pq = 0;
            (void)h2;
            const uint8_t* src = c.dbase + my_lo;
            U128u nxt{0, 0, 0, 0};
            if (nvalid) {
                uint32_t hist = 0;
                if (doc_abs + my_lo >= 4) hist = load_u32_unaligned(src - 4);
                else for (uint32_t i = 1; i <= 3 && i <= doc_abs + my_lo; i++) hist |= (uint32_t)src[-(int)i] << (32 - 8 * i);
                nxt = *reinterpret_cast<const U128u*>(src);
                if (my_lo >= 1) h1 = lgrp[hist >> 24];
                if (my_lo >= 2) h2 = lgrp[(hist >> 16) & 0xFF];
                if (my_lo >= 3) h3 = lgrp[(hist >> 8) & 0xFF];
            }
            pq = mad24s(h2, G, h1);
            mark(0);
            uint32_t acc = 0, njobs = 0, hib = 0;
            const bool want_fold = P.fold && P.nonascii;
            const uint32_t ndw = C >> 2;
            const uint32_t npieces = (ndw + 3) >> 2;
            for (uint32_t q = 0; q < npieces; q++) {
                const uint32_t w[4] = {nxt.x, nxt.y, nxt.z, nxt.w};
                if (q * 16 < nvalid) hib |= (w[0] | w[1]) | (w[2] | w[3]);
                if constexpr (SG) {
                    if (want_fold && !told_nonascii)
                        fold_job_push(q * 16 < nvalid && (((w[0] | w[1]) | (w[2] | w[3])) & 0x80808080u) != 0, lane * C + q * 16, cand, P.cand_cap, njobs);
                }
                if (q + 1 < npieces && (q + 1) * 16 < nvalid) nxt = *reinterpret_cast<const U128u*>(src + (q + 1) * 16);
                const uint32_t nd = ndw - 4 * q;
                auto dword = [&](uint32_t wd) {
                    const uint32_t c0 = lgrp[wd & 0xFF], c1 = lgrp[(wd >> 8) & 0xFF], c2 = lgrp[(wd >> 16) & 0xFF], c3 = lgrp[wd >> 24];
                    const uint32_t xa = mad24s(pq, G, c0);
                    const uint32_t xb = mad24s(mad24s(c0, G, c1), G, c2);
                    const u32x2 fa = ldual[xa], fb = ldual[xb];
                    acc = __builtin_amdgcn_alignbit(fa.x >> h3, acc, 1);
                    acc = __builtin_amdgcn_alignbit(fa.y >> c1, acc, 1);
                    acc = __builtin_amdgcn_alignbit(fb.x >> h1, acc, 1);
                    acc = __builtin_amdgcn_alignbit(fb.y >> c3, acc, 1);
                    pq = mad24s(c2, G, c3);
                    h3 = c1; h2 = c2; h1 = c3;
                };
                if (nd >= 4) {
                    uint32_t cc[19];
                    cc[0] = h3; cc[1] = h2; cc[2] = h1;
#pragma unroll
                    for (int i = 0; i < 16; i++) cc[3 + i] = lgrp[(w[i >> 2] >> (8 * (i & 3))) & 0xFF];
                    uint32_t xk[8];
                    xk[0] = mad24s(pq, G, cc[3]);
#pragma unroll
                    for (int t = 1; t < 8; t++) xk[t] = mad24s(mad24s(cc[1 + 2 * t], G, cc[2 + 2 * t]), G, cc[3 + 2 * t]);
                    u32x2 fk[8];
#pragma unroll
                    for (int t = 0; t < 8; t++) fk[t] = ldual[xk[t]];
#pragma unroll
                    for (int t = 0; t < 8; t++) {
                        acc = __builtin_amdgcn_alignbit(fk[t].x >> cc[2 * t], acc, 1);
                        acc = __builtin_amdgcn_alignbit(fk[t].y >> cc[4 + 2 * t], acc, 1);
                    }
                    pq = mad24s(cc[17], G, cc[18]);
                    h3 = cc[16]; h2 = cc[17]; h1 = cc[18];
                } else {
                    dword(w[0]);
                    if (nd >= 2) dword(w[1]);
                    if (nd >= 3) dword(w[2]);
                }
                if ((q & 1) && nd >= 4) {
                    if ((q >> 1) == 0) m0 = acc; else if ((q >> 1) == 1) m1 = acc; else if ((q >> 1) == 2) m2 = acc; else m3 = acc;
                }
            }
            if (ndw & 7) {
                const uint32_t v = acc >> (32 - 4 * (ndw & 7));
                const uint32_t k = ndw >> 3;
                if (k == 0) m0 = v; else if (k == 1) m1 = v; else if (k == 2) m2 = v; else m3 = v;
            }
            if (!SG && want_fold && !told_nonascii && __any((hib & 0x80808080u) != 0)) {
                for (uint32_t q = 0; q < npieces; q++)
                    fold_job_push((hib & 0x80808080u) != 0 && q * 16 < nvalid, lane * C + q * 16, cand, P.cand_cap, njobs);
            }
            if (njobs && !told_nonascii) {
                uint32_t bits = 1u;
                if (njobs <= P.cand_cap) {
                    FOLD_JOB_VARS(fj_);
                    bits = fold_jobs_begin(P.text, end_v, doc_abs + un.lo, own, un.lo == 0, cand, njobs, FOLD_JOB_PASS(fj_)) || fold_jobs_finish(FOLD_JOB_PASS(fj_)) ? 2u : 0u;
                }
                if (bits) { told_nonascii = true; if (lane == 0) atomicOr(P.nonascii, bits); }
            }
            m0 = nvalid >= 32 ? m0 : (nvalid ? m0 & ((1u << nvalid) - 1) : 0);
            m1 = nvalid >= 64 ? m1 : (nvalid > 32 ? m1 & ((1u << (nvalid - 32)) - 1) : 0);
            m2 = nvalid >= 96 ? m2 : (nvalid > 64 ? m2 & ((1u << (nvalid - 64)) - 1) : 0);
            m3 = nvalid >= 128 ? m3 : (nvalid > 96 ? m3 & ((1u << (nvalid - 96)) - 1) : 0);
        }
        mark(1);
        if (more_units) { abs_n = P.doc_off[un_n.doc]; end_n = P.doc_off[un_n.doc + 1]; }

        if (DBG && P.dbg) {
            if (P.dbg & 2) {
                uint32_t f = __popc(m0) + __popc(m1) + __popc(m2) + __popc(m3);
                for (int s = 32; s; s >>= 1) f += __shfl_xor(f, s, 64);
                if (lane == 0) atomicAdd(reinterpret_cast<unsigned long long*>(KARG(dbg_counters)), (unsigned long long)f);
            }
            if (P.dbg & 1) m0 = m1 = m2 = m3 = 0;
        }

        const uint32_t f = __popc(m0) + __popc(m1) + __popc(m2) + __popc(m3) + (lane == 0 ? nborder : 0);
        const uint32_t fincl = wave_incl_scan(f);
        const uint32_t ftotal = lane_value(fincl, 63);
        for (uint32_t walk = 0; walk < 2 && ftotal; walk++) {
            o.nf = 0; o.npend = 0; o.lost = false;
            for (uint32_t l0 = 0; l0 < 64;) {
                const uint32_t before = l0 ? lane_value(fincl, l0 - 1) : 0;
                const bool fits = lane >= l0 && fincl - before <= P.cand_cap;
                const uint64_t fm = __ballot(fits) >> l0;
                const uint32_t nl = fm == ~0ull >> l0 ? 64 - l0 : (uint32_t)__builtin_ctzll(~fm);
                const uint32_t l1 = l0 + nl;
                const uint32_t ptotal = lane_value(fincl, l1 - 1) - before;
                if (lane >= l0 && lane < l1) {
                    uint32_t wpos = fincl - f - before;
                    if (lane == 0)
                        for (uint32_t i = 0; i < nborder; i++) cand[wpos++] = (uint16_t)(kScan2MaxOff - nborder + i);
                    uint32_t mm[4] = {m0, m1, m2, m3};
                    const uint32_t rel = lane * C + kScan2MaxOff;
#pragma unroll
                    for (int k = 0; k < 4; k++) {
                        uint32_t mk = mm[k];
                        while (mk) {
                            const uint32_t i = __builtin_ctz(mk);
                            mk &= mk - 1;
                            cand[wpos++] = (uint16_t)(rel + 32 * k + i);
                        }
                    }
                }
                wave_lds_sync();
                mark(2);
                uint32_t ns = 0;
                bool n_on[kWays5];
                uint32_t n_rel[kWays5];
                Text8 n_tx[kWays5];
                auto fetch = [&](uint32_t i0) {
#pragma unroll
                    for (int q = 0; q < kWays5; q++) {
                        const uint32_t i = i0 + 64 * q + lane;
                        n_on[q] = i < ptotal;
                        n_rel[q] = cand[n_on[q] ? i : 0];
                    }
#pragma unroll
                    for (int q = 0; q < kWays5; q++) n_tx[q] = cand_load(c, ubase + n_rel[q]);
                };
                fetch(0);
                for (uint32_t i0 = 0; i0 < ptotal; i0 += 64 * kWays5) {
                    bool on[kWays5];
                    uint32_t rel[kWays5];
                    Text8 tx[kWays5];
                    Cand k[kWays5];
#pragma unroll
                    for (int q = 0; q < kWays5; q++) { on[q] = n_on[q]; rel[q] = n_rel[q]; tx[q] = n_tx[q]; }
                    if (i0 + 64 * kWays5 < ptotal) fetch(i0 + 64 * kWays5);
#pragma unroll
                    for (int q = 0; q < kWays5; q++) {
                        cand_keys<!SG>(c, ubase + rel[q], tx[q], k[q]);
                        if (SG && P.short3_bytes) {
                            const uint32_t wq = tx[q].w, sG = P.s5_sG;
                            k[q].sid = short3[mad24s(mad24s(lsg[(wq >> 8) & 0xFF], sG, lsg[(wq >> 16) & 0xFF]), sG, lsg[wq >> 24])];
                        }
                    }
#pragma unroll
                    for (int q = 0; q < kWays5; q++) {
                        if (FPT_LDS || !bloom_lg) cand_decide<FPT_LDS>(c, k[q]);
                        else {
                            const uint32_t* bl = reinterpret_cast<const uint32_t*>(fpt);
                            const uint32_t hg = scan5_bloom_g(k[q].x, (k[q].tw >> 24) & 0xDFu, bloom_lg), hx = scan5_bloom_x(k[q].x, bloom_lg);
                            const uint32_t wg = bl[hg >> 5], wx = bl[hx >> 5];
                            k[q].go_long = false;
                            if (((wg >> (hg & 31)) | (wx >> (hx & 31))) & 1u) cand_decide<false>(c, k[q]);
                        }
                    }
#pragma unroll
                    for (int q = 0; q < kWays5; q++)
                        if (i0 + 64 * q < ptotal)
                        {
                            const uint32_t sidq = on[q] && rel[q] >= kScan2MaxOff ? k[q].sid : 0;
                            if (SG) park_short_g(c, o, lsg, ubase, rel[q], sidq); else park_short(c, o, ubase, rel[q], sidq, k[q].x3);
                        }
                    const uint64_t below = (1ull << lane) - 1;
#pragma unroll
                    for (int q = 0; q < kWays5; q++) {
                        const bool keep = on[q] && k[q].go_long;
                        const uint64_t sb = __ballot(keep);
                        if (keep) {
                            const uint32_t at = ns + (uint32_t)__popcll(sb & below);
                            cand[at] = (uint16_t)rel[q];
                            if (at < kScan5SurvX) survx[at] = k[q].x;
                        }
                        ns += (uint32_t)__popcll(sb);
                    }
                }
                wave_lds_sync();
                mark(6);
                static_assert(kScan5SurvX >= 64, "the first stage-B trip takes its keys from survx");
                const bool b_on = lane < ns;
                const uint32_t b_rel = ns ? cand[b_on ? lane : 0] : 0;
                Cand b_k;
                b_k.p = ubase + b_rel; b_k.x3 = 0; b_k.sid = 0; b_k.go_long = true; b_k.x = 0; b_k.tw = 0;
                Slot b_s0{}, b_s1{};
                Text8 b_t8{0, 0};
                Front b_fr{};
                uint32_t b_tl = 0;
                if (ns) {
                    b_k.x = survx[b_on ? lane : 0];
                    b_s0 = slot_load(&P.slots[scan2_pair_slot(b_k.x, 0, P.slot_shift, P.slot_seed)]);
                    b_s1 = slot_load(&P.slots[scan2_pair_slot(b_k.x, 1, P.slot_shift, P.slot_seed)]);
                    if (!c.near24 && !c.near_end) {
                        const U128u v1 = *reinterpret_cast<const U128u*>(c.dbase + (int64_t)b_k.p - 23);
                        const U128u v2 = *reinterpret_cast<const U128u*>(c.dbase + (int64_t)b_k.p - 7);
                        b_fr.f[4] = v1.x; b_fr.f[3] = v1.y; b_fr.f[2] = v1.z; b_fr.f[1] = v1.w;
                        b_t8.tw = v2.x; b_t8.w = v2.y;
                        b_tl = v2.z;
                    } else {
                        b_t8 = cand_load(c, b_k.p);
                        b_fr = front_load(c, b_k.p, 0);
                        b_tl = tail_load(c, b_k.p);
                    }
                }
                while (o.npend) { if (SG) short_trip_g(c, o, lsg, ubase, o.npend < 64 ? o.npend : 64); else short_trip(c, o, ubase, o.npend < 64 ? o.npend : 64); }
                if (DBG && (P.dbg & 2)) { if (lane == 0) atomicAdd(reinterpret_cast<unsigned long long*>(KARG(dbg_counters) + 2), (unsigned long long)ns); }
                mark(3);
                Deferred dfr;
                dfr.list = reinterpret_cast<uint2*>(reinterpret_cast<uint8_t*>(cand) + ((ns * 2 + 7) & ~7u));
                dfr.cap = (P.cand_cap * 2 - ((ns * 2 + 7) & ~7u)) / 8;
                dfr.n = 0;
                if (ns) {
                    b_k.tw = b_t8.tw;
                    b_fr.f[0] = b_t8.tw;
                    finish_long5(c, o, b_on, b_rel, b_k, b_s0, b_s1, b_fr, b_tl, dfr);
                }
                for (uint32_t i0 = 64; i0 < ns; i0 += 64) {
                    const bool on = i0 + lane < ns;
                    const uint32_t rel = cand[on ? i0 + lane : 0];
                    const uint32_t p = ubase + rel;
                    Cand k;
                    k.p = p; k.x3 = 0; k.sid = 0; k.go_long = true;
                    if (i0 + 64 <= kScan5SurvX) {
                        k.x = survx[on ? i0 + lane : 0];
                        const Slot s0 = slot_load(&P.slots[scan2_pair_slot(k.x, 0, P.slot_shift, P.slot_seed)]);
                        const Slot s1 = slot_load(&P.slots[scan2_pair_slot(k.x, 1, P.slot_shift, P.slot_seed)]);
                        const Text8 t8 = cand_load(c, p);
                        const Front fr = front_load(c, p, t8.tw);
                        const uint32_t tl5 = tail_load(c, p);
                        k.tw = t8.tw;
                        finish_long5(c, o, on, rel, k, s0, s1, fr, tl5, dfr);
                    } else {
                        const Text8 t8 = cand_load(c, p);
                        const Front fr = front_load(c, p, t8.tw);
                        const uint32_t tl5 = tail_load(c, p);
                        cand_keys<false>(c, p, t8, k);
                        const Slot s0 = slot_load(&P.slots[scan2_pair_slot(k.x, 0, P.slot_shift, P.slot_seed)]);
                        const Slot s1 = slot_load(&P.slots[scan2_pair_slot(k.x, 1, P.slot_shift, P.slot_seed)]);
                        finish_long5(c, o, on, rel, k, s0, s1, fr, tl5, dfr);
                    }
                }
                if (dfr.n) drain_deferred5(c, o, ubase, dfr);
                wave_lds_sync();
                l0 = l1;
                mark(4);
            }
            if (o.direct || !o.lost) break;
            {
                const uint32_t nh = o.nf;
                if (nh > slab_left) {
                    const uint32_t want = nh > KARG(slab) ? nh : KARG(slab);
                    uint64_t nb = 0;
                    if (lane == 0) nb = atomicAdd(reinterpret_cast<unsigned long long*>(KARG(cursor)), (unsigned long long)want);
                    slab_next = static_slabs() + __shfl(nb, 0, 64);
                    slab_left = want;
                }
                o.dbase = slab_next;
                o.direct = true;
                if (slab_next + nh > KARG(pool_cap)) break;
            }
        }
        if (ftotal) {
            const uint32_t nh = o.nf;
            if (!o.direct && nh > slab_left) {
                const uint32_t want = nh > KARG(slab) ? nh : KARG(slab);
                uint64_t nb = 0;
                if (lane == 0) nb = atomicAdd(reinterpret_cast<unsigned long long*>(KARG(cursor)), (unsigned long long)want);
                slab_next = static_slabs() + __shfl(nb, 0, 64);
                slab_left = want;
            }
            const uint64_t base = slab_next;
            slab_next += nh;
            slab_left -= nh;
            wave_matches += nh;
            const bool room = base + nh <= KARG(pool_cap);
            if (lane == 0) { KARG(unit_start)[u] = base; KARG(unit_count)[u] = room ? nh : 0u; }
            if (room && !o.direct) {
                const uint32_t tmask = (1u << o.term_bits) - 1u;
                for (uint32_t i = lane; i < nh; i += 64) {
                    const uint32_t e = fifo[i];
                    if (P.want_pos) {
                        __builtin_nontemporal_store(e & tmask, &KARG(pool_term)[base + i]);
                        __builtin_nontemporal_store(o.pos_base + (e >> o.term_bits), &KARG(pool_pos)[base + i]);
                    } else {
                        __builtin_nontemporal_store(e, &KARG(pool_term)[base + i]);
                    }
                }
            }
            __builtin_amdgcn_wave_barrier();
            mark(5);
        } else if (lane == 0) {
            KARG(unit_start)[u] = slab_next; KARG(unit_count)[u] = 0;
        }
    }
    if (lane == 0) {
        if (wave_matches)
            __hip_atomic_fetch_add(reinterpret_cast<unsigned long long*>(wg_next + 2), (unsigned long long)wave_matches, __ATOMIC_RELAXED,
                                   __HIP_MEMORY_SCOPE_WORKGROUP);
        const uint32_t done = __hip_atomic_fetch_add(wg_next + 1, 1u, __ATOMIC_ACQ_REL, __HIP_MEMORY_SCOPE_WORKGROUP) & 0x7FFFFFFFu;
        if (done + 1 == kScan5Waves) {
            const unsigned long long all = __hip_atomic_load(reinterpret_cast<unsigned long long*>(wg_next + 2), __ATOMIC_RELAXED,
                                                             __HIP_MEMORY_SCOPE_WORKGROUP);
            if (all) atomicAdd(reinterpret_cast<unsigned long long*>(KARG(n_matches)), all);
        }
    }
    if (DBG && (P.dbg & 64) && lane == 0 && KARG(dbg_counters)) {
        unsigned long long all = 0;
        for (int ph = 0; ph < 8; ph++) { atomicAdd(reinterpret_cast<unsigned long long*>(KARG(dbg_counters) + 4 + ph), tl[ph]); all += tl[ph]; }
        atomicMax(reinterpret_cast<unsigned long long*>(KARG(dbg_counters) + 12), all);
        atomicAdd(reinterpret_cast<unsigned long long*>(KARG(dbg_counters) + 13), 1ull);
    }
}

}

static size_t scan5_fixed_lds(uint32_t dual_entries, uint32_t short3_bytes, uint32_t shorts_words, uint32_t fpt_lds_bytes) {
    return ((768 + (size_t)dual_entries * 8 + short3_bytes + fpt_lds_bytes + (size_t)shorts_words * 4 + 15) & ~(size_t)15) + 16;
}
static size_t scan5_wave_lds(uint32_t fifo_cap, uint32_t cand_cap) {
    return (size_t)fifo_cap * 4 + kScan5SurvX * 4 + (((size_t)cand_cap * 2 + 15) & ~(size_t)15);
}

bool scan5_plan(uint32_t kp, uint32_t short3_bytes, uint32_t shorts_words, uint32_t fpt_lds_bytes, size_t lds_max, uint32_t fifo_cap, Scan5Plan* out) {
    const uint32_t g_hi = kp < kScan5MaxGroups ? kp : kScan5MaxGroups;
    const uint32_t g_lo = g_hi > 8 + 12 ? g_hi - 8 : (g_hi < 12 ? g_hi : 12);
    for (uint32_t G = g_hi; G >= g_lo; G--) {
        const uint32_t ent = G * G * G;
        const size_t fixed = scan5_fixed_lds(ent, short3_bytes, shorts_words, fpt_lds_bytes);
        const size_t need = fixed + (size_t)kScan5Waves * scan5_wave_lds(fifo_cap, kScan5CandCapMin);
        if (need > lds_max) continue;
        const size_t spare = ((lds_max - need) / kScan5Waves / 2) & ~(size_t)7;
        out->G = G; out->dual_entries = ent;
        out->cand_cap = (uint32_t)std::min<size_t>(kScan5CandCapMin + spare, 2048);
        out->fifo_cap = fifo_cap;
        return true;
    }
    return false;
}

hipError_t launch_scan5(const Scan2Params& P, unsigned n_cus, hipStream_t st) {
    if (!P.n_units) return hipSuccess;
    const bool fl = P.fpt_lg == 0;
    const size_t lds = scan5_fixed_lds(P.s5_dual, P.short3_bytes, P.shorts_words, fl ? kScan2FptSize : P.s5_bloom_lg ? (1u << P.s5_bloom_lg) / 8 : 0) +
                       (size_t)kScan5Waves * scan5_wave_lds(P.s5_fifo_cap, P.cand_cap);
    using Kern = void (*)(const Scan2Params);
#ifdef GFT_S5_SG_CLOCKS
    const Kern fn = P.s5_sG ? (P.dbg && fl ? k_scan5<true, true, true> : fl ? k_scan5<true, false, true> : k_scan5<false, false, true>)
#else
    const Kern fn = P.s5_sG ? (fl ? k_scan5<true, false, true> : k_scan5<false, false, true>)
#endif
                    : P.dbg ? (fl ? k_scan5<true, true, false> : k_scan5<false, true, false>) : (fl ? k_scan5<true, false, false> : k_scan5<false, false, false>);
    hipError_t e = hipFuncSetAttribute(reinterpret_cast<const void*>(fn), hipFuncAttributeMaxDynamicSharedMemorySize, (int)lds);
    if (e != hipSuccess) return e;
    uint64_t g = (P.n_units + kScan5Waves - 1) / kScan5Waves;
    const unsigned grid = (unsigned)(g < n_cus ? (g ? g : 1) : n_cus);
    fn<<<dim3(grid), dim3(kScan5Waves * 64), lds, st>>>(P);
    return hipGetLastError();
}

}
```

Before: 286.4 million docs/s.

## Batch several scan units per wave item in scan5 filter passes

The scan5 kernel now has each wave take an item of K consecutive units and pack them into a shared filter pass, spreading lanes across the units in proportion to their byte counts. Before, each unit occupied a whole wave on its own. K adapts from the mean unit size, with an environment override. The aim is to keep lanes busy when units are short (about 4 KB documents) and to spread per-unit setup cost over more bytes. The price is extra wave scans and ballots per pass, a more complex lane-to-unit mapping, and possibly more divergence in the later candidate stages.

```diff
diff --git a/gofindthem_amd/csrc/gft_api.cpp b/gofindthem_amd/csrc/gft_api.cpp
--- a/gofindthem_amd/csrc/gft_api.cpp
+++ b/gofindthem_amd/csrc/gft_api.cpp
@@ -106,8 +106,10 @@
     uint32_t opt_scan5_large = 1;
     uint32_t opt_scan5_fifo = 0;
     uint32_t opt_scan5_groups = 0;
+    uint32_t opt_scan5_items = 0;
     uint64_t scan_valid_docs = ~0ull;
     uint32_t scan2_unit_max = kScan2UnitMax;
+    uint32_t scan5_item_units = 2;
     bool deferred = false;
     uint64_t deferred_unit_cap = 0, deferred_pool_cap = 0;
     uint32_t last_nonascii_bits = 0;
@@ -186,6 +188,11 @@
 
 namespace {
 
+void adapt_item_units(gft_engine* e, uint64_t text_bytes, uint64_t n_units) {
+    const uint64_t mean = std::max<uint64_t>(1, text_bytes / n_units);
+    e->scan5_item_units = (uint32_t)std::min<uint64_t>(kScan5ItemUnitsMax, std::max<uint64_t>(1, 64ull * kScan5LaneCap / mean));
+}
+
 void refresh_options(gft_engine* e) {
     auto num = [](const char* name, long dflt) { const char* v = getenv(name); return v ? atol(v) : dflt; };
     e->opt_scan_dbg = (uint32_t)num("GFT_SCAN_DEBUG", 0);
@@ -194,6 +201,7 @@
     e->opt_scan4_chunk = (uint32_t)num("GFT_SCAN4_CHUNK", 0);
     e->opt_scan4_round = (uint32_t)num("GFT_SCAN4_ROUND", 0);
     e->opt_scan5_groups = (uint32_t)num("GFT_SCAN5_GROUPS", 0);
+    e->opt_scan5_items = (uint32_t)std::min<long>(std::max<long>(num("GFT_SCAN5_ITEM_UNITS", 0), 0), kScan5ItemUnitsMax);
     e->opt_scan5_large = num("GFT_SCAN5_LARGE", 1) ? 1u : 0u;
     e->opt_scan5_bloom_kb = (uint32_t)std::min<long>(std::max<long>(num("GFT_SCAN5_BLOOM_KB", 32), 0), 64);
     e->opt_scan5_fifo = (uint32_t)std::min<long>(std::max<long>(num("GFT_SCAN5_FIFO", 0), 0), 4096) & ~63u;
@@ -697,7 +705,9 @@
             P.s5_bloom = e->s5_bloom_lg ? e->d_s5_bloom.as<uint32_t>() : nullptr; P.s5_bloom_lg = e->s5_bloom_lg;
             const uint64_t n_waves5 = (uint64_t)e->n_cus * kScan5Waves;
             P.slab = (uint32_t)std::min<uint64_t>(kScan2Slab, std::max<uint64_t>(64, e->pool_cap / (2 * n_waves5)));
-            e->last_static_slabs = std::min<uint64_t>(std::max<uint64_t>((n_units + kScan5Waves - 1) / kScan5Waves, 1), e->n_cus) * kScan5Waves * P.slab;
+            P.s5_item_units = e->opt_scan5_items ? e->opt_scan5_items : e->scan5_item_units;
+            const uint64_t n_items = (n_units + P.s5_item_units - 1) / P.s5_item_units;
+            e->last_static_slabs = std::min<uint64_t>(std::max<uint64_t>((n_items + kScan5Waves - 1) / kScan5Waves, 1), e->n_cus) * kScan5Waves * P.slab;
             ProfScope ps(e, "scan");
             HIP_TRY(launch_scan5(P, e->n_cus, st), "scan kernel launch");
         } else {
@@ -721,6 +731,9 @@
             for (int k = 4; k < 12; k++) sum += (double)t[k];
             if (t[13]) fprintf(stderr, "[gft scan debug] %llu waves: mean %.0f cycles in all, the slowest %.0f (+%.1f %%)\n", (unsigned long long)t[13],
                                sum / (double)t[13], (double)t[12], 100.0 * ((double)t[12] * (double)t[13] / sum - 1.0));
+            if (e->use_scan5 && t[14])
+                fprintf(stderr, "[gft scan debug] scan5: %llu units in %llu filter passes (up to %u units per item): per pass first bytes %.0f, filter %.0f, unit records %.0f cycles\n",
+                        (unsigned long long)n_units, (unsigned long long)t[14], P.s5_item_units, (double)t[4] / t[14], (double)t[5] / t[14], (double)t[11] / t[14]);
         }
         if (e->deferred) return GFT_OK;
         uint64_t ct[3] = {0, 0, 0};
@@ -744,6 +757,7 @@
                 uint32_t um = want >= kScan2UnitMax ? kScan2UnitMax : (uint32_t)want & ~255u;
                 e->scan2_unit_max = std::max<uint32_t>(512, um);
             }
+            if (e->use_scan5 && n_units && text_hi > text_lo && text_hi != ~0ull) adapt_item_units(e, text_hi - text_lo, n_units);
             break;
         }
         if (attempt == 2) return fail(e, GFT_E_HIP, "match pool overflow persisted");
@@ -829,6 +843,7 @@
         const uint32_t um = want >= kScan2UnitMax ? kScan2UnitMax : (uint32_t)want & ~255u;
         e->scan2_unit_max = std::max<uint32_t>(512, um);
     }
+    if (e->use_scan5 && n_units && text_hi > text_lo) adapt_item_units(e, text_hi - text_lo, n_units);
     return GFT_OK;
 }
 
diff --git a/gofindthem_amd/csrc/gft_kernels.hpp b/gofindthem_amd/csrc/gft_kernels.hpp
--- a/gofindthem_amd/csrc/gft_kernels.hpp
+++ b/gofindthem_amd/csrc/gft_kernels.hpp
@@ -240,6 +240,7 @@
     uint32_t s5_term_bits, s5_pos_bias;
     const uint32_t* s5_bloom;
     uint32_t s5_bloom_lg;
+    uint32_t s5_item_units;
 };
 GFT_HD inline uint32_t scan5_bloom_g(uint32_t x, uint32_t b1n, uint32_t lg) {
     return (scan2_mul24c<0xC2B2AFu>(x ^ (x >> 20)) + scan2_mul24c<0x27D4EBu>(b1n + 1)) >> (32 - lg);
@@ -257,6 +258,8 @@
 constexpr uint32_t kScan5MaxGroups = 27;
 constexpr uint32_t kScan5SurvX = 64;
 constexpr uint32_t kScan5CandCapMin = 384;
+constexpr uint32_t kScan5LaneCap = 160;
+constexpr uint32_t kScan5ItemUnitsMax = 16;
 struct Scan5Plan { uint32_t G, dual_entries, cand_cap, fifo_cap; };
 bool scan5_plan(uint32_t kp, uint32_t short3_bytes, uint32_t shorts_words, uint32_t fpt_lds_bytes, size_t lds_max, uint32_t fifo_cap, Scan5Plan* out);
 hipError_t launch_scan5(const Scan2Params& P, unsigned n_cus, hipStream_t st);
diff --git a/gofindthem_amd/csrc/gft_scan5.hip b/gofindthem_amd/csrc/gft_scan5.hip
--- a/gofindthem_amd/csrc/gft_scan5.hip
+++ b/gofindthem_amd/csrc/gft_scan5.hip
@@ -250,6 +250,7 @@
     auto mark = [&](int ph) {
         if (DBG && (P.dbg & 64)) { const unsigned long long now = clock64(); tl[ph] += now - tprev; tprev = now; }
     };
+    uint32_t n_iters = 0;
     auto static_slabs = [&]() { return (uint64_t)gridDim.x * kScan5Waves * KARG(slab); };
     uint64_t slab_next = ((uint64_t)blockIdx.x * kScan5Waves + wave) * KARG(slab);
     uint32_t wave_matches = 0;
@@ -257,348 +258,395 @@
     uint32_t slab_left = KARG(slab);
 
     constexpr uint32_t wg_waves = kScan5Waves;
-    const uint64_t round_units = (uint64_t)gridDim.x * wg_waves, wg_first = (uint64_t)blockIdx.x * wg_waves;
-    auto unit_of = [&](uint32_t item) -> uint64_t { return (uint64_t)(item / wg_waves) * round_units + wg_first + item % wg_waves; };
-    uint64_t u = unit_of(wave), nu = 0;
+    const uint32_t K = __builtin_amdgcn_readfirstlane(P.s5_item_units);
+    const uint64_t n_items = (P.n_units + K - 1) / K;
+    const uint64_t round_items = (uint64_t)gridDim.x * wg_waves, wg_first = (uint64_t)blockIdx.x * wg_waves;
+    auto item_of = [&](uint32_t ctr) -> uint64_t { return (uint64_t)(ctr / wg_waves) * round_items + wg_first + ctr % wg_waves; };
+    uint64_t it = item_of(wave), nit = 0;
     Unit un_n{0, 0, 0};
-    uint64_t abs_n = 0, end_n = 0;
-    if (u < P.n_units) { un_n = P.units[u]; abs_n = P.doc_off[un_n.doc]; end_n = P.doc_off[un_n.doc + 1]; }
-    for (; u < P.n_units; u = nu) {
-        const Unit un{(uint32_t)__builtin_amdgcn_readfirstlane(un_n.doc), (uint32_t)__builtin_amdgcn_readfirstlane(un_n.lo),
-                      (uint32_t)__builtin_amdgcn_readfirstlane(un_n.hi)};
-        const uint64_t doc_abs = (uint64_t)(uint32_t)__builtin_amdgcn_readfirstlane((uint32_t)(abs_n >> 32)) << 32 |
-                                 (uint32_t)__builtin_amdgcn_readfirstlane((uint32_t)abs_n);
-        const uint64_t end_v = end_n;
+    uint64_t abs_n = 0;
+    uint32_t dlen_n = 0;
+    if (it < n_items && lane < K && it * K + lane < P.n_units) {
+        un_n = P.units[it * K + lane]; abs_n = P.doc_off[un_n.doc]; dlen_n = (uint32_t)(P.doc_off[un_n.doc + 1] - abs_n);
+    }
+    for (; it < n_items; it = nit) {
+        const uint64_t u0 = it * K;
+        const uint32_t nK = (uint32_t)(P.n_units - u0 < K ? P.n_units - u0 : K);
+        const uint32_t i_lo = un_n.lo, i_hi = un_n.hi;
+        const uint64_t i_abs = abs_n;
+        const uint32_t i_dlen = dlen_n;
         {
-            uint32_t item = 0;
-            if (lane == 0) item = __hip_atomic_fetch_add(wg_next, 1u, __ATOMIC_RELAXED, __HIP_MEMORY_SCOPE_WORKGROUP);
-            nu = unit_of((uint32_t)__builtin_amdgcn_readfirstlane(item));
+            uint32_t ctr = 0;
+            if (lane == 0) ctr = __hip_atomic_fetch_add(wg_next, 1u, __ATOMIC_RELAXED, __HIP_MEMORY_SCOPE_WORKGROUP);
+            nit = item_of((uint32_t)__builtin_amdgcn_readfirstlane(ctr));
         }
         mark(7);
-        const bool more_units = nu < P.n_units;
-        if (more_units) un_n = P.units[nu];
-        const Ctx c{P, cls, nullptr, P.short3_bytes ? short3 : nullptr, fpt, lrec, P.text + doc_abs, doc_abs, kp2,
-                    doc_abs < 7, doc_abs < 23, un.lo, un.hi, doc_abs + un.hi + 4 > P.text_bytes, DBG ? P.dbg : 0u};
-        const uint32_t nborder = un.lo < kScan2MaxOff ? un.lo : kScan2MaxOff;
-        const uint32_t ubase = un.lo - kScan2MaxOff;
-        const uint32_t own = un.hi - un.lo;
-        const uint32_t C = ((own + 63) / 64 + 3) & ~3u;
-        const uint32_t my_lo = un.lo + lane * C;
-        const uint32_t my_hi = my_lo + C < un.hi ? my_lo + C : un.hi;
-        const uint32_t nvalid = my_lo < un.hi ? my_hi - my_lo : 0;
-        Ctx5 o{fifo, P.s5_fifo_cap, 0, 0, false, false, 0, P.s5_term_bits, un.lo - P.s5_pos_bias};
-
-        uint32_t m0 = 0, m1 = 0, m2 = 0, m3 = 0;
-        if (own) {
-            uint32_t h1 = P.s5_pad_g, h2 = P.s5_pad_g, h3 = P.s5_pad_g, pq = 0;
-            (void)h2;
-            const uint8_t* src = c.dbase + my_lo;
-            U128u nxt{0, 0, 0, 0};
-            if (nvalid) {
-                uint32_t hist = 0;
-                if (doc_abs + my_lo >= 4) hist = load_u32_unaligned(src - 4);
-                else for (uint32_t i = 1; i <= 3 && i <= doc_abs + my_lo; i++) hist |= (uint32_t)src[-(int)i] << (32 - 8 * i);
-                nxt = *reinterpret_cast<const U128u*>(src);
-                if (my_lo >= 1) h1 = lgrp[hist >> 24];
-                if (my_lo >= 2) h2 = lgrp[(hist >> 16) & 0xFF];
-                if (my_lo >= 3) h3 = lgrp[(hist >> 8) & 0xFF];
+        const bool more_items = nit < n_items;
+        const bool n_mine = more_items && lane < K && nit * K + lane < P.n_units;
+        if (n_mine) un_n = P.units[nit * K + lane];
+        const uint32_t i_own = lane < nK ? i_hi - i_lo : 0u;
+
+        for (uint32_t j0 = 0; j0 < nK;) {
+            const bool cand_u = lane >= j0 && lane < nK;
+            const uint32_t need_cap = cand_u ? (i_own > kScan5LaneCap ? (i_own + kScan5LaneCap - 1) / kScan5LaneCap : 1u) : 0u;
+            const uint32_t nfit = (uint32_t)__popcll(__ballot(cand_u && wave_incl_scan(need_cap) <= 64));
+            const uint32_t j1 = j0 + (nfit ? nfit : 1u);
+            const bool in_pass = lane >= j0 && lane < j1;
+            const uint32_t pass_bytes = lane_value(wave_incl_scan(in_pass ? i_own : 0u), 63);
+            uint32_t C = ((pass_bytes + 63) / 64 + 3) & ~3u;
+            if (C == 0) C = 4;
+            uint32_t nl_u = 0, nl_incl = 0;
+            for (;;) {
+                nl_u = in_pass ? (i_own > C ? (i_own + C - 1) / C : 1u) : 0u;
+                nl_incl = wave_incl_scan(nl_u);
+                if (C >= kScan5LaneCap || lane_value(nl_incl, 63) <= 64) break;
+                C += 4;
             }
-            pq = mad24s(h2, G, h1);
-            mark(0);
-            uint32_t acc = 0, njobs = 0, hib = 0;
-            const bool want_fold = P.fold && P.nonascii;
+            const uint32_t lanes_u = (nl_incl - nl_u) | nl_incl << 8;
+            uint32_t my_lo = 0, my_hi = 0;
+            uint64_t my_abs = 0;
+            for (uint32_t j = j0; j < j1; j++) {
+                const uint32_t lj = lane_value(lanes_u, j), L = lj & 0xFFu;
+                if (lane >= L && lane < lj >> 8) {
+                    my_lo = lane_value(i_lo, j) + (lane - L) * C;
+                    my_hi = lane_value(i_hi, j);
+                    my_abs = (uint64_t)lane_value((uint32_t)(i_abs >> 32), j) << 32 | lane_value((uint32_t)i_abs, j);
+                }
+            }
+            my_hi = my_lo + C < my_hi ? my_lo + C : my_hi;
+            const uint32_t nvalid = my_lo < my_hi ? my_hi - my_lo : 0;
+            if (DBG) n_iters++;
+
+            uint32_t m0 = 0, m1 = 0, m2 = 0, m3 = 0, m4 = 0;
+            uint32_t pm = 0;
             const uint32_t ndw = C >> 2;
             const uint32_t npieces = (ndw + 3) >> 2;
-            for (uint32_t q = 0; q < npieces; q++) {
-                const uint32_t w[4] = {nxt.x, nxt.y, nxt.z, nxt.w};
-                if (q * 16 < nvalid) hib |= (w[0] | w[1]) | (w[2] | w[3]);
-                if constexpr (SG) {
-                    if (want_fold && !told_nonascii)
-                        fold_job_push(q * 16 < nvalid && (((w[0] | w[1]) | (w[2] | w[3])) & 0x80808080u) != 0, lane * C + q * 16, cand, P.cand_cap, njobs);
+            const bool want_fold = P.fold && P.nonascii;
+            if (pass_bytes) {
+                uint32_t h1 = P.s5_pad_g, h2 = P.s5_pad_g, h3 = P.s5_pad_g, pq = 0;
+                (void)h2;
+                const uint8_t* src = P.text + my_abs + my_lo;
+                U128u nxt{0, 0, 0, 0};
+                if (nvalid) {
+                    uint32_t hist = 0;
+                    if (my_abs + my_lo >= 4) hist = load_u32_unaligned(src - 4);
+                    else for (uint32_t i = 1; i <= 3 && i <= my_abs + my_lo; i++) hist |= (uint32_t)src[-(int)i] << (32 - 8 * i);
+                    nxt = *reinterpret_cast<const U128u*>(src);
+                    if (my_lo >= 1) h1 = lgrp[hist >> 24];
+                    if (my_lo >= 2) h2 = lgrp[(hist >> 16) & 0xFF];
+                    if (my_lo >= 3) h3 = lgrp[(hist >> 8) & 0xFF];
                 }
-                if (q + 1 < npieces && (q + 1) * 16 < nvalid) nxt = *reinterpret_cast<const U128u*>(src + (q + 1) * 16);
-                const uint32_t nd = ndw - 4 * q;
-                auto dword = [&](uint32_t wd) {
-                    const uint32_t c0 = lgrp[wd & 0xFF], c1 = lgrp[(wd >> 8) & 0xFF], c2 = lgrp[(wd >> 16) & 0xFF], c3 = lgrp[wd >> 24];
-                    const uint32_t xa = mad24s(pq, G, c0);
-                    const uint32_t xb = mad24s(mad24s(c0, G, c1), G, c2);
-                    const u32x2 fa = ldual[xa], fb = ldual[xb];
-                    acc = __builtin_amdgcn_alignbit(fa.x >> h3, acc, 1);
-                    acc = __builtin_amdgcn_alignbit(fa.y >> c1, acc, 1);
-                    acc = __builtin_amdgcn_alignbit(fb.x >> h1, acc, 1);
-                    acc = __builtin_amdgcn_alignbit(fb.y >> c3, acc, 1);
-                    pq = mad24s(c2, G, c3);
-                    h3 = c1; h2 = c2; h1 = c3;
-                };
-                if (nd >= 4) {
-                    uint32_t cc[19];
-                    cc[0] = h3; cc[1] = h2; cc[2] = h1;
-#pragma unroll
-                    for (int i = 0; i < 16; i++) cc[3 + i] = lgrp[(w[i >> 2] >> (8 * (i & 3))) & 0xFF];
-                    uint32_t xk[8];
-                    xk[0] = mad24s(pq, G, cc[3]);
-#pragma unroll
-                    for (int t = 1; t < 8; t++) xk[t] = mad24s(mad24s(cc[1 + 2 * t], G, cc[2 + 2 * t]), G, cc[3 + 2 * t]);
-                    u32x2 fk[8];
-#pragma unroll
-                    for (int t = 0; t < 8; t++) fk[t] = ldual[xk[t]];
-#pragma unroll
-                    for (int t = 0; t < 8; t++) {
-                        acc = __builtin_amdgcn_alignbit(fk[t].x >> cc[2 * t], acc, 1);
-                        acc = __builtin_amdgcn_alignbit(fk[t].y >> cc[4 + 2 * t], acc, 1);
+                pq = mad24s(h2, G, h1);
+                mark(0);
+                uint32_t acc = 0, hib = 0;
+                for (uint32_t q = 0; q < npieces; q++) {
+                    const uint32_t w[4] = {nxt.x, nxt.y, nxt.z, nxt.w};
+                    if (q * 16 < nvalid) hib |= (w[0] | w[1]) | (w[2] | w[3]);
+                    if constexpr (SG) {
+                        if (want_fold && q * 16 < nvalid && (((w[0] | w[1]) | (w[2] | w[3])) & 0x80808080u) != 0) pm |= 1u << q;
                     }
-                    pq = mad24s(cc[17], G, cc[18]);
-                    h3 = cc[16]; h2 = cc[17]; h1 = cc[18];
-                } else {
-                    dword(w[0]);
-                    if (nd >= 2) dword(w[1]);
-                    if (nd >= 3) dword(w[2]);
+                    if (q + 1 < npieces && (q + 1) * 16 < nvalid) nxt = *reinterpret_cast<const U128u*>(src + (q + 1) * 16);
+                    const uint32_t nd = ndw - 4 * q;
+                    auto dword = [&](uint32_t wd) {
+                        const uint32_t c0 = lgrp[wd & 0xFF], c1 = lgrp[(wd >> 8) & 0xFF], c2 = lgrp[(wd >> 16) & 0xFF], c3 = lgrp[wd >> 24];
+                        const uint32_t xa = mad24s(pq, G, c0);
+                        const uint32_t xb = mad24s(mad24s(c0, G, c1), G, c2);
+                        const u32x2 fa = ldual[xa], fb = ldual[xb];
+                        acc = __builtin_amdgcn_alignbit(fa.x >> h3, acc, 1);
+                        acc = __builtin_amdgcn_alignbit(fa.y >> c1, acc, 1);
+                        acc = __builtin_amdgcn_alignbit(fb.x >> h1, acc, 1);
+                        acc = __builtin_amdgcn_alignbit(fb.y >> c3, acc, 1);
+                        pq = mad24s(c2, G, c3);
+                        h3 = c1; h2 = c2; h1 = c3;
+                    };
+                    if (nd >= 4) {
+                        uint32_t cc[19];
+                        cc[0] = h3; cc[1] = h2; cc[2] = h1;
+#pragma unroll
+                        for (int i = 0; i < 16; i++) cc[3 + i] = lgrp[(w[i >> 2] >> (8 * (i & 3))) & 0xFF];
+                        uint32_t xk[8];
+                        xk[0] = mad24s(pq, G, cc[3]);
+#pragma unroll
+                        for (int t = 1; t < 8; t++) xk[t] = mad24s(mad24s(cc[1 + 2 * t], G, cc[2 + 2 * t]), G, cc[3 + 2 * t]);
+                        u32x2 fk[8];
+#pragma unroll
+                        for (int t = 0; t < 8; t++) fk[t] = ldual[xk[t]];
+#pragma unroll
+                        for (int t = 0; t < 8; t++) {
+                            acc = __builtin_amdgcn_alignbit(fk[t].x >> cc[2 * t], acc, 1);
+                            acc = __builtin_amdgcn_alignbit(fk[t].y >> cc[4 + 2 * t], acc, 1);
+                        }
+                        pq = mad24s(cc[17], G, cc[18]);
+                        h3 = cc[16]; h2 = cc[17]; h1 = cc[18];
+                    } else {
+                        dword(w[0]);
+                        if (nd >= 2) dword(w[1]);
+                        if (nd >= 3) dword(w[2]);
+                    }
+                    if ((q & 1) && nd >= 4) {
+                        const uint32_t k = q >> 1;
+                        if (k == 0) m0 = acc; else if (k == 1) m1 = acc; else if (k == 2) m2 = acc; else if (k == 3) m3 = acc; else m4 = acc;
+                    }
                 }
-                if ((q & 1) && nd >= 4) {
-                    if ((q >> 1) == 0) m0 = acc; else if ((q >> 1) == 1) m1 = acc; else if ((q >> 1) == 2) m2 = acc; else m3 = acc;
+                if (ndw & 7) {
+                    const uint32_t v = acc >> (32 - 4 * (ndw & 7));
+                    const uint32_t k = ndw >> 3;
+                    if (k == 0) m0 = v; else if (k == 1) m1 = v; else if (k == 2) m2 = v; else if (k == 3) m3 = v; else m4 = v;
+                }
+                if (!SG && want_fold && (hib & 0x80808080u) != 0)
+                    for (uint32_t q = 0; q < npieces; q++) pm |= (q * 16 < nvalid ? 1u : 0u) << q;
+                m0 = nvalid >= 32 ? m0 : (nvalid ? m0 & ((1u << nvalid) - 1) : 0);
+                m1 = nvalid >= 64 ? m1 : (nvalid > 32 ? m1 & ((1u << (nvalid - 32)) - 1) : 0);
+                m2 = nvalid >= 96 ? m2 : (nvalid > 64 ? m2 & ((1u << (nvalid - 64)) - 1) : 0);
+                m3 = nvalid >= 128 ? m3 : (nvalid > 96 ? m3 & ((1u << (nvalid - 96)) - 1) : 0);
+                m4 = nvalid >= 160 ? m4 : (nvalid > 128 ? m4 & ((1u << (nvalid - 128)) - 1) : 0);
+            }
+            mark(1);
+            if (j0 == 0 && n_mine) { abs_n = P.doc_off[un_n.doc]; dlen_n = (uint32_t)(P.doc_off[un_n.doc + 1] - abs_n); }
+
+            if (DBG && P.dbg) {
+                if (P.dbg & 2) {
+                    uint32_t f = __popc(m0) + __popc(m1) + __popc(m2) + __popc(m3) + __popc(m4);
+                    for (int s = 32; s; s >>= 1) f += __shfl_xor(f, s, 64);
+                    if (lane == 0) atomicAdd(reinterpret_cast<unsigned long long*>(KARG(dbg_counters)), (unsigned long long)f);
+                }
+                if (P.dbg & 1) m0 = m1 = m2 = m3 = m4 = 0;
+            }
+
+            for (uint32_t j = j0; j < j1; j++) {
+                const uint64_t u = u0 + j;
+                const uint32_t lj = lane_value(lanes_u, j), L_lo = lj & 0xFFu, L_hi = lj >> 8;
+                const bool mine = lane >= L_lo && lane < L_hi;
+                const Unit un{0, lane_value(i_lo, j), lane_value(i_hi, j)};
+                const uint64_t doc_abs = (uint64_t)lane_value((uint32_t)(i_abs >> 32), j) << 32 | lane_value((uint32_t)i_abs, j);
+                const Ctx c{P, cls, nullptr, P.short3_bytes ? short3 : nullptr, fpt, lrec, P.text + doc_abs, doc_abs, kp2,
+                            doc_abs < 7, doc_abs < 23, un.lo, un.hi, doc_abs + un.hi + 4 > P.text_bytes, DBG ? P.dbg : 0u};
+                const uint32_t nborder = un.lo < kScan2MaxOff ? un.lo : kScan2MaxOff;
+                const uint32_t ubase = un.lo - kScan2MaxOff;
+                const uint32_t own = un.hi - un.lo;
+                Ctx5 o{fifo, P.s5_fifo_cap, 0, 0, false, false, 0, P.s5_term_bits, un.lo - P.s5_pos_bias};
+
+                if (want_fold && !told_nonascii && __any(mine && pm != 0)) {
+                    uint32_t njobs = 0;
+                    for (uint32_t q = 0; q < npieces; q++) fold_job_push(mine && (pm >> q & 1u), (lane - L_lo) * C + q * 16, cand, P.cand_cap, njobs);
+                    uint32_t bits = 1u;
+                    if (njobs <= P.cand_cap) {
+                        FOLD_JOB_VARS(fj_);
+                        bits = fold_jobs_begin(P.text, doc_abs + lane_value(i_dlen, j), doc_abs + un.lo, own, un.lo == 0, cand, njobs, FOLD_JOB_PASS(fj_)) || fold_jobs_finish(FOLD_JOB_PASS(fj_)) ? 2u : 0u;
+                    }
+                    if (bits) { told_nonascii = true; if (lane == 0) atomicOr(P.nonascii, bits); }
+                }
+
+                const uint32_t f = mine ? __popc(m0) + __popc(m1) + __popc(m2) + __popc(m3) + __popc(m4) + (lane == L_lo ? nborder : 0) : 0u;
+                const uint32_t fincl = wave_incl_scan(f);
+                const uint32_t ftotal = lane_value(fincl, 63);
+                for (uint32_t walk = 0; walk < 2 && ftotal; walk++) {
+                    o.nf = 0; o.npend = 0; o.lost = false;
+                    for (uint32_t l0 = L_lo; l0 < L_hi;) {
+                        const uint32_t before = l0 ? lane_value(fincl, l0 - 1) : 0;
+                        const bool fits = lane >= l0 && fincl - before <= P.cand_cap;
+                        const uint64_t fm = __ballot(fits) >> l0;
+                        const uint32_t nl = fm == ~0ull >> l0 ? 64 - l0 : (uint32_t)__builtin_ctzll(~fm);
+                        const uint32_t l1 = l0 + nl;
+                        const uint32_t ptotal = lane_value(fincl, l1 - 1) - before;
+                        if (mine && lane >= l0 && lane < l1) {
+                            uint32_t wpos = fincl - f - before;
+                            if (lane == L_lo)
+                                for (uint32_t i = 0; i < nborder; i++) cand[wpos++] = (uint16_t)(kScan2MaxOff - nborder + i);
+                            uint32_t mm[5] = {m0, m1, m2, m3, m4};
+                            const uint32_t rel = (lane - L_lo) * C + kScan2MaxOff;
+#pragma unroll
+                            for (int k = 0; k < 5; k++) {
+                                uint32_t mk = mm[k];
+                                while (mk) {
+                                    const uint32_t i = __builtin_ctz(mk);
+                                    mk &= mk - 1;
+                                    cand[wpos++] = (uint16_t)(rel + 32 * k + i);
+                                }
+                            }
+                        }
+                        wave_lds_sync();
+                        mark(2);
+                        uint32_t ns = 0;
+                        bool n_on[kWays5];
+                        uint32_t n_rel[kWays5];
+                        Text8 n_tx[kWays5];
+                        auto fetch = [&](uint32_t i0) {
+#pragma unroll
+                            for (int q = 0; q < kWays5; q++) {
+                                const uint32_t i = i0 + 64 * q + lane;
+                                n_on[q] = i < ptotal;
+                                n_rel[q] = cand[n_on[q] ? i : 0];
+                            }
+#pragma unroll
+                            for (int q = 0; q < kWays5; q++) n_tx[q] = cand_load(c, ubase + n_rel[q]);
+                        };
+                        if (ptotal) fetch(0);
+                        for (uint32_t i0 = 0; i0 < ptotal; i0 += 64 * kWays5) {
+                            bool on[kWays5];
+                            uint32_t rel[kWays5];
+                            Text8 tx[kWays5];
+                            Cand k[kWays5];
+#pragma unroll
+                            for (int q = 0; q < kWays5; q++) { on[q] = n_on[q]; rel[q] = n_rel[q]; tx[q] = n_tx[q]; }
+                            if (i0 + 64 * kWays5 < ptotal) fetch(i0 + 64 * kWays5);
+#pragma unroll
+                            for (int q = 0; q < kWays5; q++) {
+                                cand_keys<!SG>(c, ubase + rel[q], tx[q], k[q]);
+                                if (SG && P.short3_bytes) {
+                                    const uint32_t wq = tx[q].w, sG = P.s5_sG;
+                                    k[q].sid = short3[mad24s(mad24s(lsg[(wq >> 8) & 0xFF], sG, lsg[(wq >> 16) & 0xFF]), sG, lsg[wq >> 24])];
+                                }
+                            }
+#pragma unroll
+                            for (int q = 0; q < kWays5; q++) {
+                                if (FPT_LDS || !bloom_lg) cand_decide<FPT_LDS>(c, k[q]);
+                                else {
+                                    const uint32_t* bl = reinterpret_cast<const uint32_t*>(fpt);
+                                    const uint32_t hg = scan5_bloom_g(k[q].x, (k[q].tw >> 24) & 0xDFu, bloom_lg), hx = scan5_bloom_x(k[q].x, bloom_lg);
+                                    const uint32_t wg = bl[hg >> 5], wx = bl[hx >> 5];
+                                    k[q].go_long = false;
+                                    if (((wg >> (hg & 31)) | (wx >> (hx & 31))) & 1u) cand_decide<false>(c, k[q]);
+                                }
+                            }
+#pragma unroll
+                            for (int q = 0; q < kWays5; q++)
+                                if (i0 + 64 * q < ptotal)
+                                {
+                                    const uint32_t sidq = on[q] && rel[q] >= kScan2MaxOff ? k[q].sid : 0;
+                                    if (SG) park_short_g(c, o, lsg, ubase, rel[q], sidq); else park_short(c, o, ubase, rel[q], sidq, k[q].x3);
+                                }
+                            const uint64_t below = (1ull << lane) - 1;
+#pragma unroll
+                            for (int q = 0; q < kWays5; q++) {
+                                const bool keep = on[q] && k[q].go_long;
+                                const uint64_t sb = __ballot(keep);
+                                if (keep) {
+                                    const uint32_t at = ns + (uint32_t)__popcll(sb & below);
+                                    cand[at] = (uint16_t)rel[q];
+                                    if (at < kScan5SurvX) survx[at] = k[q].x;
+                                }
+                                ns += (uint32_t)__popcll(sb);
+                            }
+                        }
+                        wave_lds_sync();
+                        mark(6);
+                        static_assert(kScan5SurvX >= 64, "the first stage-B trip takes its keys from survx");
+                        const bool b_on = lane < ns;
+                        const uint32_t b_rel = ns ? cand[b_on ? lane : 0] : 0;
+                        Cand b_k;
+                        b_k.p = ubase + b_rel; b_k.x3 = 0; b_k.sid = 0; b_k.go_long = true; b_k.x = 0; b_k.tw = 0;
+                        Slot b_s0{}, b_s1{};
+                        Text8 b_t8{0, 0};
+                        Front b_fr{};
+                        uint32_t b_tl = 0;
+                        if (ns) {
+                            b_k.x = survx[b_on ? lane : 0];
+                            b_s0 = slot_load(&P.slots[scan2_pair_slot(b_k.x, 0, P.slot_shift, P.slot_seed)]);
+                            b_s1 = slot_load(&P.slots[scan2_pair_slot(b_k.x, 1, P.slot_shift, P.slot_seed)]);
+                            if (!c.near24 && !c.near_end) {
+                                const U128u v1 = *reinterpret_cast<const U128u*>(c.dbase + (int64_t)b_k.p - 23);
+                                const U128u v2 = *reinterpret_cast<const U128u*>(c.dbase + (int64_t)b_k.p - 7);
+                                b_fr.f[4] = v1.x; b_fr.f[3] = v1.y; b_fr.f[2] = v1.z; b_fr.f[1] = v1.w;
+                                b_t8.tw = v2.x; b_t8.w = v2.y;
+                                b_tl = v2.z;
+                            } else {
+                                b_t8 = cand_load(c, b_k.p);
+                                b_fr = front_load(c, b_k.p, 0);
+                                b_tl = tail_load(c, b_k.p);
+                            }
+                        }
+                        while (o.npend) { if (SG) short_trip_g(c, o, lsg, ubase, o.npend < 64 ? o.npend : 64); else short_trip(c, o, ubase, o.npend < 64 ? o.npend : 64); }
+                        if (DBG && (P.dbg & 2)) { if (lane == 0) atomicAdd(reinterpret_cast<unsigned long long*>(KARG(dbg_counters) + 2), (unsigned long long)ns); }
+                        mark(3);
+                        Deferred dfr;
+                        dfr.list = reinterpret_cast<uint2*>(reinterpret_cast<uint8_t*>(cand) + ((ns * 2 + 7) & ~7u));
+                        dfr.cap = (P.cand_cap * 2 - ((ns * 2 + 7) & ~7u)) / 8;
+                        dfr.n = 0;
+                        if (ns) {
+                            b_k.tw = b_t8.tw;
+                            b_fr.f[0] = b_t8.tw;
+                            finish_long5(c, o, b_on, b_rel, b_k, b_s0, b_s1, b_fr, b_tl, dfr);
+                        }
+                        for (uint32_t i0 = 64; i0 < ns; i0 += 64) {
+                            const bool on = i0 + lane < ns;
+                            const uint32_t rel = cand[on ? i0 + lane : 0];
+                            const uint32_t p = ubase + rel;
+                            Cand k;
+                            k.p = p; k.x3 = 0; k.sid = 0; k.go_long = true;
+                            if (i0 + 64 <= kScan5SurvX) {
+                                k.x = survx[on ? i0 + lane : 0];
+                                const Slot s0 = slot_load(&P.slots[scan2_pair_slot(k.x, 0, P.slot_shift, P.slot_seed)]);
+                                const Slot s1 = slot_load(&P.slots[scan2_pair_slot(k.x, 1, P.slot_shift, P.slot_seed)]);
+                                const Text8 t8 = cand_load(c, p);
+                                const Front fr = front_load(c, p, t8.tw);
+                                const uint32_t tl5 = tail_load(c, p);
+                                k.tw = t8.tw;
+                                finish_long5(c, o, on, rel, k, s0, s1, fr, tl5, dfr);
+                            } else {
+                                const Text8 t8 = cand_load(c, p);
+                                const Front fr = front_load(c, p, t8.tw);
+                                const uint32_t tl5 = tail_load(c, p);
+                                cand_keys<false>(c, p, t8, k);
+                                const Slot s0 = slot_load(&P.slots[scan2_pair_slot(k.x, 0, P.slot_shift, P.slot_seed)]);
+                                const Slot s1 = slot_load(&P.slots[scan2_pair_slot(k.x, 1, P.slot_shift, P.slot_seed)]);
+                                finish_long5(c, o, on, rel, k, s0, s1, fr, tl5, dfr);
+                            }
+                        }
+                        if (dfr.n) drain_deferred5(c, o, ubase, dfr);
+                        wave_lds_sync();
+                        l0 = l1;
+                        mark(4);
+                    }
+                    if (o.direct || !o.lost) break;
+                    {
+                        const uint32_t nh = o.nf;
+                        if (nh > slab_left) {
+                            const uint32_t want = nh > KARG(slab) ? nh : KARG(slab);
+                            uint64_t nb = 0;
+                            if (lane == 0) nb = atomicAdd(reinterpret_cast<unsigned long long*>(KARG(cursor)), (unsigned long long)want);
+                            slab_next = static_slabs() + __shfl(nb, 0, 64);
+                            slab_left = want;
+                        }
+                        o.dbase = slab_next;
+                        o.direct = true;
+                        if (slab_next + nh > KARG(pool_cap)) break;
+                    }
+                }
+                if (ftotal) {
+                    const uint32_t nh = o.nf;
+                    if (!o.direct && nh > slab_left) {
+                        const uint32_t want = nh > KARG(slab) ? nh : KARG(slab);
+                        uint64_t nb = 0;
+                        if (lane == 0) nb = atomicAdd(reinterpret_cast<unsigned long long*>(KARG(cursor)), (unsigned long long)want);
+                        slab_next = static_slabs() + __shfl(nb, 0, 64);
+                        slab_left = want;
+                    }
+                    const uint64_t base = slab_next;
+                    slab_next += nh;
+                    slab_left -= nh;
+                    wave_matches += nh;
+                    const bool room = base + nh <= KARG(pool_cap);
+                    if (lane == 0) { KARG(unit_start)[u] = base; KARG(unit_count)[u] = room ? nh : 0u; }
+                    if (room && !o.direct) {
+                        const uint32_t tmask = (1u << o.term_bits) - 1u;
+                        for (uint32_t i = lane; i < nh; i += 64) {
+                            const uint32_t e = fifo[i];
+                            if (P.want_pos) {
+                                __builtin_nontemporal_store(e & tmask, &KARG(pool_term)[base + i]);
+                                __builtin_nontemporal_store(o.pos_base + (e >> o.term_bits), &KARG(pool_pos)[base + i]);
+                            } else {
+                                __builtin_nontemporal_store(e, &KARG(pool_term)[base + i]);
+                            }
+                        }
+                    }
+                    __builtin_amdgcn_wave_barrier();
+                    mark(5);
+                } else if (lane == 0) {
+                    KARG(unit_start)[u] = slab_next; KARG(unit_count)[u] = 0;
                 }
             }
-            if (ndw & 7) {
-                const uint32_t v = acc >> (32 - 4 * (ndw & 7));
-                const uint32_t k = ndw >> 3;
-                if (k == 0) m0 = v; else if (k == 1) m1 = v; else if (k == 2) m2 = v; else m3 = v;
-            }
-            if (!SG && want_fold && !told_nonascii && __any((hib & 0x80808080u) != 0)) {
-                for (uint32_t q = 0; q < npieces; q++)
-                    fold_job_push((hib & 0x80808080u) != 0 && q * 16 < nvalid, lane * C + q * 16, cand, P.cand_cap, njobs);
-            }
-            if (njobs && !told_nonascii) {
-                uint32_t bits = 1u;
-                if (njobs <= P.cand_cap) {
-                    FOLD_JOB_VARS(fj_);
-                    bits = fold_jobs_begin(P.text, end_v, doc_abs + un.lo, own, un.lo == 0, cand, njobs, FOLD_JOB_PASS(fj_)) || fold_jobs_finish(FOLD_JOB_PASS(fj_)) ? 2u : 0u;
-                }
-                if (bits) { told_nonascii = true; if (lane == 0) atomicOr(P.nonascii, bits); }
-            }
-            m0 = nvalid >= 32 ? m0 : (nvalid ? m0 & ((1u << nvalid) - 1) : 0);
-            m1 = nvalid >= 64 ? m1 : (nvalid > 32 ? m1 & ((1u << (nvalid - 32)) - 1) : 0);
-            m2 = nvalid >= 96 ? m2 : (nvalid > 64 ? m2 & ((1u << (nvalid - 64)) - 1) : 0);
-            m3 = nvalid >= 128 ? m3 : (nvalid > 96 ? m3 & ((1u << (nvalid - 96)) - 1) : 0);
-        }
-        mark(1);
-        if (more_units) { abs_n = P.doc_off[un_n.doc]; end_n = P.doc_off[un_n.doc + 1]; }
-
-        if (DBG && P.dbg) {
-            if (P.dbg & 2) {
-                uint32_t f = __popc(m0) + __popc(m1) + __popc(m2) + __popc(m3);
-                for (int s = 32; s; s >>= 1) f += __shfl_xor(f, s, 64);
-                if (lane == 0) atomicAdd(reinterpret_cast<unsigned long long*>(KARG(dbg_counters)), (unsigned long long)f);
-            }
-            if (P.dbg & 1) m0 = m1 = m2 = m3 = 0;
-        }
-
-        const uint32_t f = __popc(m0) + __popc(m1) + __popc(m2) + __popc(m3) + (lane == 0 ? nborder : 0);
-        const uint32_t fincl = wave_incl_scan(f);
-        const uint32_t ftotal = lane_value(fincl, 63);
-        for (uint32_t walk = 0; walk < 2 && ftotal; walk++) {
-            o.nf = 0; o.npend = 0; o.lost = false;
-            for (uint32_t l0 = 0; l0 < 64;) {
-                const uint32_t before = l0 ? lane_value(fincl, l0 - 1) : 0;
-                const bool fits = lane >= l0 && fincl - before <= P.cand_cap;
-                const uint64_t fm = __ballot(fits) >> l0;
-                const uint32_t nl = fm == ~0ull >> l0 ? 64 - l0 : (uint32_t)__builtin_ctzll(~fm);
-                const uint32_t l1 = l0 + nl;
-                const uint32_t ptotal = lane_value(fincl, l1 - 1) - before;
-                if (lane >= l0 && lane < l1) {
-                    uint32_t wpos = fincl - f - before;
-                    if (lane == 0)
-                        for (uint32_t i = 0; i < nborder; i++) cand[wpos++] = (uint16_t)(kScan2MaxOff - nborder + i);
-                    uint32_t mm[4] = {m0, m1, m2, m3};
-                    const uint32_t rel = lane * C + kScan2MaxOff;
-#pragma unroll
-                    for (int k = 0; k < 4; k++) {
-                        uint32_t mk = mm[k];
-                        while (mk) {
-                            const uint32_t i = __builtin_ctz(mk);
-                            mk &= mk - 1;
-                            cand[wpos++] = (uint16_t)(rel + 32 * k + i);
-                        }
-                    }
-                }
-                wave_lds_sync();
-                mark(2);
-                uint32_t ns = 0;
-                bool n_on[kWays5];
-                uint32_t n_rel[kWays5];
-                Text8 n_tx[kWays5];
-                auto fetch = [&](uint32_t i0) {
-#pragma unroll
-                    for (int q = 0; q < kWays5; q++) {
-                        const uint32_t i = i0 + 64 * q + lane;
-                        n_on[q] = i < ptotal;
-                        n_rel[q] = cand[n_on[q] ? i : 0];
-                    }
-#pragma unroll
-                    for (int q = 0; q < kWays5; q++) n_tx[q] = cand_load(c, ubase + n_rel[q]);
-                };
-                fetch(0);
-                for (uint32_t i0 = 0; i0 < ptotal; i0 += 64 * kWays5) {
-                    bool on[kWays5];
-                    uint32_t rel[kWays5];
-                    Text8 tx[kWays5];
-                    Cand k[kWays5];
-#pragma unroll
-                    for (int q = 0; q < kWays5; q++) { on[q] = n_on[q]; rel[q] = n_rel[q]; tx[q] = n_tx[q]; }
-                    if (i0 + 64 * kWays5 < ptotal) fetch(i0 + 64 * kWays5);
-#pragma unroll
-                    for (int q = 0; q < kWays5; q++) {
-                        cand_keys<!SG>(c, ubase + rel[q], tx[q], k[q]);
-                        if (SG && P.short3_bytes) {
-                            const uint32_t wq = tx[q].w, sG = P.s5_sG;
-                            k[q].sid = short3[mad24s(mad24s(lsg[(wq >> 8) & 0xFF], sG, lsg[(wq >> 16) & 0xFF]), sG, lsg[wq >> 24])];
-                        }
-                    }
-#pragma unroll
-                    for (int q = 0; q < kWays5; q++) {
-                        if (FPT_LDS || !bloom_lg) cand_decide<FPT_LDS>(c, k[q]);
-                        else {
-                            const uint32_t* bl = reinterpret_cast<const uint32_t*>(fpt);
-                            const uint32_t hg = scan5_bloom_g(k[q].x, (k[q].tw >> 24) & 0xDFu, bloom_lg), hx = scan5_bloom_x(k[q].x, bloom_lg);
-                            const uint32_t wg = bl[hg >> 5], wx = bl[hx >> 5];
-                            k[q].go_long = false;
-                            if (((wg >> (hg & 31)) | (wx >> (hx & 31))) & 1u) cand_decide<false>(c, k[q]);
-                        }
-                    }
-#pragma unroll
-                    for (int q = 0; q < kWays5; q++)
-                        if (i0 + 64 * q < ptotal)
-                        {
-                            const uint32_t sidq = on[q] && rel[q] >= kScan2MaxOff ? k[q].sid : 0;
-                            if (SG) park_short_g(c, o, lsg, ubase, rel[q], sidq); else park_short(c, o, ubase, rel[q], sidq, k[q].x3);
-                        }
-                    const uint64_t below = (1ull << lane) - 1;
-#pragma unroll
-                    for (int q = 0; q < kWays5; q++) {
-                        const bool keep = on[q] && k[q].go_long;
-                        const uint64_t sb = __ballot(keep);
-                        if (keep) {
-                            const uint32_t at = ns + (uint32_t)__popcll(sb & below);
-                            cand[at] = (uint16_t)rel[q];
-                            if (at < kScan5SurvX) survx[at] = k[q].x;
-                        }
-                        ns += (uint32_t)__popcll(sb);
-                    }
-                }
-                wave_lds_sync();
-                mark(6);
-                static_assert(kScan5SurvX >= 64, "the first stage-B trip takes its keys from survx");
-                const bool b_on = lane < ns;
-                const uint32_t b_rel = ns ? cand[b_on ? lane : 0] : 0;
-                Cand b_k;
-                b_k.p = ubase + b_rel; b_k.x3 = 0; b_k.sid = 0; b_k.go_long = true; b_k.x = 0; b_k.tw = 0;
-                Slot b_s0{}, b_s1{};
-                Text8 b_t8{0, 0};
-                Front b_fr{};
-                uint32_t b_tl = 0;
-                if (ns) {
-                    b_k.x = survx[b_on ? lane : 0];
-                    b_s0 = slot_load(&P.slots[scan2_pair_slot(b_k.x, 0, P.slot_shift, P.slot_seed)]);
-                    b_s1 = slot_load(&P.slots[scan2_pair_slot(b_k.x, 1, P.slot_shift, P.slot_seed)]);
-                    if (!c.near24 && !c.near_end) {
-                        const U128u v1 = *reinterpret_cast<const U128u*>(c.dbase + (int64_t)b_k.p - 23);
-                        const U128u v2 = *reinterpret_cast<const U128u*>(c.dbase + (int64_t)b_k.p - 7);
-                        b_fr.f[4] = v1.x; b_fr.f[3] = v1.y; b_fr.f[2] = v1.z; b_fr.f[1] = v1.w;
-                        b_t8.tw = v2.x; b_t8.w = v2.y;
-                        b_tl = v2.z;
-                    } else {
-                        b_t8 = cand_load(c, b_k.p);
-                        b_fr = front_load(c, b_k.p, 0);
-                        b_tl = tail_load(c, b_k.p);
-                    }
-                }
-                while (o.npend) { if (SG) short_trip_g(c, o, lsg, ubase, o.npend < 64 ? o.npend : 64); else short_trip(c, o, ubase, o.npend < 64 ? o.npend : 64); }
-                if (DBG && (P.dbg & 2)) { if (lane == 0) atomicAdd(reinterpret_cast<unsigned long long*>(KARG(dbg_counters) + 2), (unsigned long long)ns); }
-                mark(3);
-                Deferred dfr;
-                dfr.list = reinterpret_cast<uint2*>(reinterpret_cast<uint8_t*>(cand) + ((ns * 2 + 7) & ~7u));
-                dfr.cap = (P.cand_cap * 2 - ((ns * 2 + 7) & ~7u)) / 8;
-                dfr.n = 0;
-                if (ns) {
-                    b_k.tw = b_t8.tw;
-                    b_fr.f[0] = b_t8.tw;
-                    finish_long5(c, o, b_on, b_rel, b_k, b_s0, b_s1, b_fr, b_tl, dfr);
-                }
-                for (uint32_t i0 = 64; i0 < ns; i0 += 64) {
-                    const bool on = i0 + lane < ns;
-                    const uint32_t rel = cand[on ? i0 + lane : 0];
-                    const uint32_t p = ubase + rel;
-                    Cand k;
-                    k.p = p; k.x3 = 0; k.sid = 0; k.go_long = true;
-                    if (i0 + 64 <= kScan5SurvX) {
-                        k.x = survx[on ? i0 + lane : 0];
-                        const Slot s0 = slot_load(&P.slots[scan2_pair_slot(k.x, 0, P.slot_shift, P.slot_seed)]);
-                        const Slot s1 = slot_load(&P.slots[scan2_pair_slot(k.x, 1, P.slot_shift, P.slot_seed)]);
-                        const Text8 t8 = cand_load(c, p);
-                        const Front fr = front_load(c, p, t8.tw);
-                        const uint32_t tl5 = tail_load(c, p);
-                        k.tw = t8.tw;
-                        finish_long5(c, o, on, rel, k, s0, s1, fr, tl5, dfr);
-                    } else {
-                        const Text8 t8 = cand_load(c, p);
-                        const Front fr = front_load(c, p, t8.tw);
-                        const uint32_t tl5 = tail_load(c, p);
-                        cand_keys<false>(c, p, t8, k);
-                        const Slot s0 = slot_load(&P.slots[scan2_pair_slot(k.x, 0, P.slot_shift, P.slot_seed)]);
-                        const Slot s1 = slot_load(&P.slots[scan2_pair_slot(k.x, 1, P.slot_shift, P.slot_seed)]);
-                        finish_long5(c, o, on, rel, k, s0, s1, fr, tl5, dfr);
-                    }
-                }
-                if (dfr.n) drain_deferred5(c, o, ubase, dfr);
-                wave_lds_sync();
-                l0 = l1;
-                mark(4);
-            }
-            if (o.direct || !o.lost) break;
-            {
-                const uint32_t nh = o.nf;
-                if (nh > slab_left) {
-                    const uint32_t want = nh > KARG(slab) ? nh : KARG(slab);
-                    uint64_t nb = 0;
-                    if (lane == 0) nb = atomicAdd(reinterpret_cast<unsigned long long*>(KARG(cursor)), (unsigned long long)want);
-                    slab_next = static_slabs() + __shfl(nb, 0, 64);
-                    slab_left = want;
-                }
-                o.dbase = slab_next;
-                o.direct = true;
-                if (slab_next + nh > KARG(pool_cap)) break;
-            }
-        }
-        if (ftotal) {
-            const uint32_t nh = o.nf;
-            if (!o.direct && nh > slab_left) {
-                const uint32_t want = nh > KARG(slab) ? nh : KARG(slab);
-                uint64_t nb = 0;
-                if (lane == 0) nb = atomicAdd(reinterpret_cast<unsigned long long*>(KARG(cursor)), (unsigned long long)want);
-                slab_next = static_slabs() + __shfl(nb, 0, 64);
-                slab_left = want;
-            }
-            const uint64_t base = slab_next;
-            slab_next += nh;
-            slab_left -= nh;
-            wave_matches += nh;
-            const bool room = base + nh <= KARG(pool_cap);
-            if (lane == 0) { KARG(unit_start)[u] = base; KARG(unit_count)[u] = room ? nh : 0u; }
-            if (room && !o.direct) {
-                const uint32_t tmask = (1u << o.term_bits) - 1u;
-                for (uint32_t i = lane; i < nh; i += 64) {
-                    const uint32_t e = fifo[i];
-                    if (P.want_pos) {
-                        __builtin_nontemporal_store(e & tmask, &KARG(pool_term)[base + i]);
-                        __builtin_nontemporal_store(o.pos_base + (e >> o.term_bits), &KARG(pool_pos)[base + i]);
-                    } else {
-                        __builtin_nontemporal_store(e, &KARG(pool_term)[base + i]);
-                    }
-                }
-            }
-            __builtin_amdgcn_wave_barrier();
-            mark(5);
-        } else if (lane == 0) {
-            KARG(unit_start)[u] = slab_next; KARG(unit_count)[u] = 0;
+            j0 = j1;
         }
     }
     if (lane == 0) {
@@ -617,6 +665,7 @@
         for (int ph = 0; ph < 8; ph++) { atomicAdd(reinterpret_cast<unsigned long long*>(KARG(dbg_counters) + 4 + ph), tl[ph]); all += tl[ph]; }
         atomicMax(reinterpret_cast<unsigned long long*>(KARG(dbg_counters) + 12), all);
         atomicAdd(reinterpret_cast<unsigned long long*>(KARG(dbg_counters) + 13), 1ull);
+        atomicAdd(reinterpret_cast<unsigned long long*>(KARG(dbg_counters) + 14), (unsigned long long)n_iters);
     }
 }
 
@@ -648,6 +697,7 @@
 
 hipError_t launch_scan5(const Scan2Params& P, unsigned n_cus, hipStream_t st) {
     if (!P.n_units) return hipSuccess;
+    if (P.s5_item_units < 1 || P.s5_item_units > kScan5ItemUnitsMax) return hipErrorInvalidValue;
     const bool fl = P.fpt_lg == 0;
     const size_t lds = scan5_fixed_lds(P.s5_dual, P.short3_bytes, P.shorts_words, fl ? kScan2FptSize : P.s5_bloom_lg ? (1u << P.s5_bloom_lg) / 8 : 0) +
                        (size_t)kScan5Waves * scan5_wave_lds(P.s5_fifo_cap, P.cand_cap);
@@ -660,7 +710,8 @@
                     : P.dbg ? (fl ? k_scan5<true, true, false> : k_scan5<false, true, false>) : (fl ? k_scan5<true, false, false> : k_scan5<false, false, false>);
     hipError_t e = hipFuncSetAttribute(reinterpret_cast<const void*>(fn), hipFuncAttributeMaxDynamicSharedMemorySize, (int)lds);
     if (e != hipSuccess) return e;
-    uint64_t g = (P.n_units + kScan5Waves - 1) / kScan5Waves;
+    const uint64_t n_items = (P.n_units + P.s5_item_units - 1) / P.s5_item_units;
+    uint64_t g = (n_items + kScan5Waves - 1) / kScan5Waves;
     const unsigned grid = (unsigned)(g < n_cus ? (g ? g : 1) : n_cus);
     fn<<<dim3(grid), dim3(kScan5Waves * 64), lds, st>>>(P);
     return hipGetLastError();
```

Result: slower. 246.3 million docs/s (median of 2 runs) (-14.0%).
